# DanMcGann/loam

Hardware: AMD Instinct MI355X
Metric: scan-pair registrations/sec (64x1024 Ouster) (higher is better)
Workload: dtype f64; 1 GPU; batch of 1024 independent 64x1024 scan pairs per GPU (BASELINE configs[2]/[3]); step = extractFeatures x2 + registerFeatures per pair, inputs resident in HBM; pairs_per_gpu=1024, scan=64x1024, seed=20240311, input_scalar=f64, arithmetic=f64 (float input is widened on load)

## Files before the change

### loam_amd/csrc/loamx_api.hip

```cpp
#include <math.h>
#include <stdio.h>
#include <stdlib.h>
#include <string.h>

#include <mutex>
#include <utility>
#include <string>
#include <vector>

#include <dlfcn.h>
#include <rccl/rccl.h>

#include "loamx_internal.h"
#include "synth.h"

using namespace loamx;

namespace {

enum WsId {
  WS_XYZ = 0, WS_CURV, WS_MASK, WS_EDGE_STAGE, WS_PLANAR_STAGE, WS_EDGE_CNT, WS_PLANAR_CNT,
  WS_EDGE_IDX, WS_PLANAR_IDX, WS_N_EDGE, WS_N_PLANAR, WS_EDGE_XYZ, WS_PLANAR_XYZ,
  WS_GRID_DESC_E, WS_GRID_DESC_P, WS_CELLS_E, WS_CELLS_P, WS_SORTED_E, WS_SORTED_P, WS_REL_E, WS_REL_P,
  WS_SGRID_DESC_E, WS_SGRID_DESC_P, WS_SCELLS_E, WS_SCELLS_P, WS_SSORTED_E, WS_SSORTED_P, WS_SORT_SCRATCH, WS_SORT_SCRATCH_SRC, WS_ASSOC_E, WS_ASSOC_P, WS_NN_E, WS_NN_P, WS_RNN_E, WS_RNN_P, WS_NEAREST_E, WS_NEAREST_P, WS_REST_E, WS_REST_P, WS_EXACT_E, WS_EXACT_P, WS_NASSOC, WS_STATE, WS_PARTIALS, WS_MOM_PARTIALS, WS_MOMENTS, WS_FLAGGED_LIST, WS_FLAGGED_COUNT, WS_LINE_TOT, WS_EXTRACT_EVENTS, WS_BOX, WS_FINITE_FLAG,
  WS_COUNTERS, WS_ITERINFO, WS_STREAM_IN0, WS_STREAM_IN1, WS_STREAM_RES, WS_DUMP_E, WS_DUMP_P, WS_FIT_IN, WS_FIT_OUT, WS_SRC_E, WS_SRC_P, WS_TGT_E, WS_TGT_P, WS_FCOUNTS, WS_RESULTS, WS_INIT,
  WS_COUNT
};

struct Buf {
  void* p = nullptr;
  size_t cap = 0;
};

struct PendingEvent {
  int kernel;
  hipEvent_t e0, e1;
  double bytes;
  bool own_e0;
};

}

struct loamx_ctx {
  int device = 0;
  hipStream_t own_stream = nullptr, stream = nullptr;
  bool max_counts_clean = false;
  hipStream_t aux_stream = nullptr;
  hipEvent_t ev_fork = nullptr, ev_mid = nullptr, ev_join = nullptr;
  hipEvent_t ev_counts = nullptr;
  hipStream_t aux2_stream = nullptr;
  hipEvent_t ev_join2 = nullptr;
  std::string last_error;
  Buf ws[WS_COUNT];
  uint32_t* h_pinned = nullptr;
  bool timing = false;
  std::vector<PendingEvent> pending;
  std::vector<hipEvent_t> event_pool;
  hipEvent_t tail_event = nullptr;
  bool tail_fresh = false;
  loamx_kernel_stat stats[LOAMX_K_COUNT] = {};

  uint32_t extract_flags = 0;
  uint32_t reg_flags = 0;
  int map_cells_log2 = 0;
  int stream_chunk_pairs = 0;
  hipStream_t copy_stream = nullptr;
  hipEvent_t ev_up[2] = {nullptr, nullptr}, ev_free[2] = {nullptr, nullptr};

  unsigned long long sweep_slots_base[2] = {0, 0};
  unsigned long long features_base = 0;
  std::mutex mu;
};

struct loamx_target_index {
  GridDesc* desc[2] = {nullptr, nullptr};
  uint32_t* cells[2] = {nullptr, nullptr};
  GridPoint* sorted[2] = {nullptr, nullptr};
  float* rel[2] = {nullptr, nullptr};
  double* pts[2] = {nullptr, nullptr};
  size_t n[2] = {0, 0};
  size_t cap[2] = {0, 0};
  double radius[2] = {0, 0};
  uint32_t* counts = nullptr;
  void* scratch = nullptr;
  uint32_t cells_cap[2] = {0, 0};
  size_t cells_alloc[2] = {0, 0}, scratch_alloc = 0;
  GridPoint* sorted2[2] = {nullptr, nullptr};
  float* rel2[2] = {nullptr, nullptr};
  size_t n_at_build[2] = {0, 0};
  bool grid_valid[2] = {false, false};
  uint64_t full_builds = 0, merges = 0;
};

namespace loamx {
thread_local LaunchScope* g_launch_scope = nullptr;
int g_debug_sync = getenv("LOAMX_DEBUG_SYNC") ? 1 : 0;
}

namespace {

const char* kKernelNames[LOAMX_K_COUNT] = {"curvature_valid_kernel", "select_kernel", "compact_kernel",
                                           "grid_build_kernel",      "associate_kernel", "sweep_kernel",
                                           "lm_kernels",             "moment_kernel",    "knn_plane_kernel",
                                           "extract_fused_kernel"};

struct OptionName {
  const char* name;
  bool extract;
  uint32_t bit;
};
const OptionName kOptionNames[] = {
    {"FORCE_TIE_REPLAY", true, kFlagForceReplay}, {"FORCE_SCAN_GIVEUP", true, kFlagForceGiveUp}, {"CURV_V1", true, kFlagCurvV1},
    {"NO_FUSED_COMPACT", true, kFlagNoFusedCompact}, {"NO_MIS_SELECT", true, kFlagNoMisSelect}, {"FUSED_EXTRACT", true, kFlagFusedExtract},
    {"NO_ROW_SELECT", true, kFlagNoRowSelect}, {"FUSED_ROWS", true, kFlagFusedRows}, {"NO_SPLIT_CURV", true, kFlagNoSplitCurv}, {"STAGE_ALWAYS", true, kFlagStageAlways},
    {"NO_MOMENTS", false, kRegFlagNoMoments}, {"NO_PACKED_GRID", false, kRegFlagNoPackedGrid}, {"NO_BIG_GRID", false, kRegFlagNoBigGrid},
    {"NO_GRID_SIDE", false, kRegFlagNoGridSide}, {"DEBUG_POISON", false, kRegFlagPoison},
    {"QUEUE_TWO_STAGE", false, kRegFlagQueueTwoStage}, {"QUEUE_ONE_STAGE", false, kRegFlagQueueOneStage},
    {"NO_MIXED_ASSOC", false, kRegFlagNoMixedAssoc}, {"FORCE_RCCL", false, kRegFlagForceRccl},
    {"NO_COOP_LEFT", false, kRegFlagNoCoopLeft}, {"NO_REF_MOMENTS", false, kRegFlagNoRefMoments},
    {"NO_EXTRACT_BOXES", false, kRegFlagNoExtractBoxes}, {"CHECK_FINITE", false, kRegFlagCheckFinite},
    {"NO_SMALL_SETS", false, kRegFlagNoSmallSets}};

int fail(loamx_ctx* ctx, int code, const std::string& msg) {
  if (ctx) ctx->last_error = msg;
  return code;
}

#define HIP_TRY(ctx, expr)                                                                          \
  do {                                                                                              \
    hipError_t e_ = (expr);                                                                         \
    if (e_ != hipSuccess)                                                                           \
      return fail(ctx, LOAMX_ERR_HIP, std::string(#expr) + ": " + hipGetErrorString(e_));           \
  } while (0)

int ensure(loamx_ctx* ctx, int id, size_t bytes) {
  Buf& b = ctx->ws[id];
  if (bytes == 0) bytes = 8;
  if (b.cap >= bytes) return LOAMX_OK;
  if (b.p) {
    HIP_TRY(ctx, hipStreamSynchronize(ctx->stream));
    HIP_TRY(ctx, hipFree(b.p));
    b.p = nullptr, b.cap = 0;
  }
  HIP_TRY(ctx, hipMalloc(&b.p, bytes));
  b.cap = bytes;
  return LOAMX_OK;
}
#define ENSURE(ctx, id, bytes)                       \
  do {                                               \
    int rc_ = ensure(ctx, id, bytes);                \
    if (rc_ != LOAMX_OK) return rc_;                 \
  } while (0)

const char* const kNonFiniteMsg = "non-finite coordinate in the input (the reference's behaviour is undefined there)";
bool host_all_finite(const void* p, bool f32, size_t n_scalars) {
  if (!p) return true;
  if (f32) {
    const float* v = static_cast<const float*>(p);
    float acc = 0.0f;
    for (size_t i = 0; i < n_scalars; i++) acc += v[i] * 0.0f;
    return acc == 0.0f;
  }
  const double* v = static_cast<const double*>(p);
  double acc = 0.0;
  for (size_t i = 0; i < n_scalars; i++) acc += v[i] * 0.0;
  return acc == 0.0;
}
template <typename T>
T* wsp(loamx_ctx* ctx, int id) {
  return reinterpret_cast<T*>(ctx->ws[id].p);
}

hipEvent_t take_event(loamx_ctx* ctx) {
  if (!ctx->event_pool.empty()) {
    hipEvent_t e = ctx->event_pool.back();
    ctx->event_pool.pop_back();
    return e;
  }
  hipEvent_t e = nullptr;
  (void)hipEventCreate(&e);
  return e;
}

struct TimedScope {
  loamx_ctx* ctx;
  PendingEvent pe;
  bool on, attach;
  LaunchScope ls;
  TimedScope(loamx_ctx* c, int kernel, double bytes, bool attach_ = false) : ctx(c), on(c->timing), attach(attach_) {
    if (on) {
      pe.kernel = kernel, pe.bytes = bytes;
      if (attach) {
        pe.own_e0 = true;
        pe.e0 = take_event(ctx), pe.e1 = take_event(ctx);
        ls = LaunchScope{pe.e0, pe.e1, true};
        g_launch_scope = &ls;
        return;
      }
      pe.own_e0 = !(ctx->tail_fresh && ctx->tail_event);
      pe.e0 = pe.own_e0 ? take_event(ctx) : ctx->tail_event;
      pe.e1 = take_event(ctx);
      if (pe.own_e0) (void)hipEventRecord(pe.e0, ctx->stream);
    }
  }
// ... 278 lines not shown
    }
    if (it > 0 || ref_first) {
      TimedScope t(ctx, LOAMX_K_MOMENT, 0.0, true);
      launch_moments(B, s);
    }
    if (it > 0 || ref_first) {
      TimedScope t(ctx, LOAMX_K_LM, 0.0, true);
      launch_lm_pair_loop(B, C, s);
    } else {
      for (int k = 0; k < 5; k++) {
        {
          TimedScope t(ctx, LOAMX_K_SWEEP, 0.0, true);
          launch_sweep(B, s);
        }
        {
          TimedScope t(ctx, LOAMX_K_LM, 0.0, true);
          launch_lm_step(B, s);
        }
      }
    }
    CHECK_LAUNCH(ctx, "sweep/lm kernels");
    if (it == 0 && !ref_first) {
      TimedScope t(ctx, LOAMX_K_LM, 0.0, true);
      launch_outer_update(B, C, s);
    }
    CHECK_LAUNCH(ctx, "outer_update_kernel");
  return LOAMX_OK;
}

int register_dev(loamx_ctx* ctx, const RegInputs& in, const RegConfig& C_in, loamx_reg_result* d_results, bool want_iter_info,
                 AfterAssocHook hook, void* hook_user, const loamx_target_index* prebuilt = nullptr, const loamx_assoc_dump* dump = nullptr,
                 size_t dump_n_se = 0, size_t dump_n_sp = 0) {
  if (in.n_pairs == 0) return LOAMX_OK;
  RegConfig C = C_in;
  if (dump && C.max_iterations == 0) C.max_iterations = 1;
  untimed(ctx);
  if (in.n_pairs > 0x7FFFFFFFull / 128) return fail(ctx, LOAMX_ERR_UNSUPPORTED, "too many pairs in one call");
  const size_t np = in.n_pairs, es = in.edge_stride ? in.edge_stride : 1, ps = in.planar_stride ? in.planar_stride : 1;
  if (es > 0x3FFFFFFFull || ps > 0x3FFFFFFFull) return fail(ctx, LOAMX_ERR_UNSUPPORTED, "feature set too large");
  RegBatch B{};
  B.n_pairs = np, B.edge_stride = es, B.planar_stride = ps, B.in_pitch = in.in_pitch;
  B.src_edge = in.src_edge, B.n_src_edge = in.n_src_edge, B.src_planar = in.src_planar, B.n_src_planar = in.n_src_planar;
  B.tgt_edge = in.tgt_edge, B.n_tgt_edge = in.n_tgt_edge, B.tgt_planar = in.tgt_planar, B.n_tgt_planar = in.n_tgt_planar;
  B.init = in.init;
  if (!(C.flags & kRegFlagNoExtractBoxes)) B.box_min = in.boxes.min, B.box_max = in.boxes.max, B.box_bad = in.boxes.bad;
  ENSURE(ctx, WS_GRID_DESC_E, np * sizeof(GridDesc));
  ENSURE(ctx, WS_GRID_DESC_P, np * sizeof(GridDesc));
  ENSURE(ctx, WS_CELLS_E, (np * (size_t)(kGridCellsCap + 1) + 4) * sizeof(uint32_t));
  ENSURE(ctx, WS_CELLS_P, (np * (size_t)(kGridCellsCap + 1) + 4) * sizeof(uint32_t));
  ENSURE(ctx, WS_SORTED_E, np * (es + kGridPad) * sizeof(GridPoint));
  ENSURE(ctx, WS_SORTED_P, np * (ps + kGridPad) * sizeof(GridPoint));
  ENSURE(ctx, WS_REL_E, np * 3 * (es + kGridPad) * sizeof(float));
  ENSURE(ctx, WS_REL_P, np * 3 * (ps + kGridPad) * sizeof(float));
  ENSURE(ctx, WS_SGRID_DESC_E, np * sizeof(GridDesc));
  ENSURE(ctx, WS_SGRID_DESC_P, np * sizeof(GridDesc));
  ENSURE(ctx, WS_SCELLS_E, np * (size_t)(kGridCellsCap + 1) * sizeof(uint32_t));
  ENSURE(ctx, WS_SCELLS_P, np * (size_t)(kGridCellsCap + 1) * sizeof(uint32_t));
  ENSURE(ctx, WS_SSORTED_E, np * es * sizeof(GridPoint));
  ENSURE(ctx, WS_SSORTED_P, np * ps * sizeof(GridPoint));
  ENSURE(ctx, WS_SORT_SCRATCH, np * (es > ps ? es : ps) * sizeof(GridPoint));
  ENSURE(ctx, WS_SORT_SCRATCH_SRC, grid_small(es > ps ? es : ps, C.flags) ? sizeof(GridPoint) : np * (es > ps ? es : ps) * sizeof(GridPoint));
  ENSURE(ctx, WS_ASSOC_E, 9 * np * es * sizeof(double));
  ENSURE(ctx, WS_ASSOC_P, 7 * np * ps * sizeof(double));
  const size_t km_e = C.k_edge <= 5 ? 5 : (C.k_edge <= 8 ? 8 : kMaxK), km_p = C.k_plane <= 5 ? 5 : (C.k_plane <= 8 ? 8 : kMaxK);
  ENSURE(ctx, WS_NN_E, (1 + km_e) * np * es * sizeof(uint32_t));
  ENSURE(ctx, WS_NN_P, (1 + km_p) * np * ps * sizeof(uint32_t));
  ENSURE(ctx, WS_RNN_E, (1 + km_e) * np * es * sizeof(uint32_t));
  ENSURE(ctx, WS_RNN_P, (1 + km_p) * np * ps * sizeof(uint32_t));
  ENSURE(ctx, WS_NEAREST_E, np * es * sizeof(uint32_t));
  ENSURE(ctx, WS_NEAREST_P, np * ps * sizeof(uint32_t));
  ENSURE(ctx, WS_REST_E, np * es * sizeof(uint32_t));
  ENSURE(ctx, WS_REST_P, np * ps * sizeof(uint32_t));
  ENSURE(ctx, WS_EXACT_E, np * es * sizeof(uint32_t));
  ENSURE(ctx, WS_EXACT_P, np * ps * sizeof(uint32_t));
  ENSURE(ctx, WS_NASSOC, np * 8 * sizeof(uint32_t));
  ENSURE(ctx, WS_STATE, np * sizeof(PairState));
  B.blocks_per_pair = (uint32_t)((es + ps + kSweepChunk - 1) / kSweepChunk);
  ENSURE(ctx, WS_PARTIALS, np * B.blocks_per_pair * kAccSize * sizeof(double));
  B.mom_blocks_per_pair = (uint32_t)((ps + kSweepChunk - 1) / kSweepChunk);
  ENSURE(ctx, WS_MOM_PARTIALS, np * B.mom_blocks_per_pair * 4 * (size_t)(kMomSize + 2) * sizeof(double));
  ENSURE(ctx, WS_MOMENTS, np * (size_t)(kMomSize + 2) * sizeof(double));
  ENSURE(ctx, WS_FLAGGED_LIST, np * (size_t)B.mom_blocks_per_pair * kSweepChunk * sizeof(uint32_t));
  ENSURE(ctx, WS_FLAGGED_COUNT, np * (size_t)B.mom_blocks_per_pair * 4 * sizeof(uint32_t));
  {
    const bool fresh = ctx->ws[WS_COUNTERS].cap == 0;
    ENSURE(ctx, WS_COUNTERS, 128);
    untimed(ctx);
    if (fresh) HIP_TRY(ctx, hipMemsetAsync(ctx->ws[WS_COUNTERS].p, 0, 128, ctx->stream));
  }
  if (C.flags & kRegFlagPoison) {
    static const int kScratch[] = {WS_GRID_DESC_E, WS_GRID_DESC_P, WS_CELLS_E, WS_CELLS_P, WS_SORTED_E, WS_SORTED_P, WS_REL_E, WS_REL_P,
                                   WS_SGRID_DESC_E, WS_SGRID_DESC_P, WS_SCELLS_E, WS_SCELLS_P, WS_SSORTED_E, WS_SSORTED_P, WS_SORT_SCRATCH, WS_SORT_SCRATCH_SRC,
                                   WS_ASSOC_E, WS_ASSOC_P, WS_NN_E, WS_NN_P, WS_RNN_E, WS_RNN_P, WS_NEAREST_E, WS_NEAREST_P, WS_REST_E,
                                   WS_REST_P, WS_EXACT_E, WS_EXACT_P, WS_NASSOC, WS_STATE, WS_PARTIALS, WS_MOM_PARTIALS, WS_MOMENTS,
                                   WS_FLAGGED_LIST, WS_FLAGGED_COUNT};
    for (int id : kScratch)
      if (ctx->ws[id].p) HIP_TRY(ctx, hipMemsetAsync(ctx->ws[id].p, 0xFF, ctx->ws[id].cap, ctx->stream));
  }
  if (want_iter_info) ENSURE(ctx, WS_ITERINFO, np * (size_t)(C.max_iterations ? C.max_iterations : 1) * sizeof(loamx_iter_info));
  B.grid_edge = GridSet{wsp<GridDesc>(ctx, WS_GRID_DESC_E), wsp<uint32_t>(ctx, WS_CELLS_E), wsp<GridPoint>(ctx, WS_SORTED_E), es + kGridPad,
                        wsp<float>(ctx, WS_REL_E)};
  B.grid_plane = GridSet{wsp<GridDesc>(ctx, WS_GRID_DESC_P), wsp<uint32_t>(ctx, WS_CELLS_P), wsp<GridPoint>(ctx, WS_SORTED_P), ps + kGridPad,
                         wsp<float>(ctx, WS_REL_P)};
  B.src_grid_edge = GridSet{wsp<GridDesc>(ctx, WS_SGRID_DESC_E), wsp<uint32_t>(ctx, WS_SCELLS_E), wsp<GridPoint>(ctx, WS_SSORTED_E), es, nullptr};
  B.src_grid_plane = GridSet{wsp<GridDesc>(ctx, WS_SGRID_DESC_P), wsp<uint32_t>(ctx, WS_SCELLS_P), wsp<GridPoint>(ctx, WS_SSORTED_P), ps, nullptr};
  B.sort_scratch = wsp<GridPoint>(ctx, WS_SORT_SCRATCH);
  B.sort_scratch_src = wsp<GridPoint>(ctx, WS_SORT_SCRATCH_SRC);
  B.assoc = AssocBuffers{wsp<double>(ctx, WS_ASSOC_E), wsp<double>(ctx, WS_ASSOC_P), wsp<uint32_t>(ctx, WS_NN_E),
                         wsp<uint32_t>(ctx, WS_NN_P), wsp<uint32_t>(ctx, WS_RNN_E), wsp<uint32_t>(ctx, WS_RNN_P),
                         wsp<uint32_t>(ctx, WS_NEAREST_E),
                         wsp<uint32_t>(ctx, WS_NEAREST_P), wsp<uint32_t>(ctx, WS_REST_E), wsp<uint32_t>(ctx, WS_REST_P),
                         wsp<uint32_t>(ctx, WS_EXACT_E), wsp<uint32_t>(ctx, WS_EXACT_P),
                         wsp<uint32_t>(ctx, WS_NASSOC)};
  B.state = wsp<PairState>(ctx, WS_STATE);
  B.partials = wsp<double>(ctx, WS_PARTIALS);
  B.mom_partials = wsp<double>(ctx, WS_MOM_PARTIALS);
  B.moments = wsp<double>(ctx, WS_MOMENTS);
  B.flagged_list = wsp<uint32_t>(ctx, WS_FLAGGED_LIST);
  B.flagged_count = wsp<uint32_t>(ctx, WS_FLAGGED_COUNT);
  B.n_active = wsp<uint32_t>(ctx, WS_COUNTERS);
  B.sweep_slots = reinterpret_cast<unsigned long long*>(wsp<unsigned char>(ctx, WS_COUNTERS) + 8);
  B.assoc_slots = B.sweep_slots + 2;
  B.grid_bytes = B.sweep_slots + 5;
  B.iter_info = want_iter_info ? wsp<loamx_iter_info>(ctx, WS_ITERINFO) : nullptr;
  B.want_nearest = hook ? 1u : 0u;
  B.ref_moments = (C.flags & (kRegFlagNoMoments | kRegFlagNoRefMoments)) ? 0u : 1u;
  B.max_counts = wsp<uint32_t>(ctx, WS_COUNTERS) + 16;
  B.assoc_blocks_edge = B.assoc_blocks_plane = 0xFFFFFFFFu;
  B.knn_mode_edge = B.knn_mode_plane = 0u;
  B.small_edge_sets = (C.flags & kRegFlagNoSmallSets) ? 0u : (!prebuilt ? 1u : (prebuilt->n[0] <= kBruteMax ? 2u : 0u));
  hipStream_t s = ctx->stream;
  untimed(ctx);
  if (!ctx->max_counts_clean) {
    const uint32_t init[6] = {0u, 0u, 0u, 0u, 0xFFFFFFFFu, 0xFFFFFFFFu};
    memcpy(&ctx->h_pinned[8], init, sizeof(init));
    HIP_TRY(ctx, hipMemcpyAsync(B.max_counts, &ctx->h_pinned[8], sizeof(init), hipMemcpyHostToDevice, s));
  }
  ctx->max_counts_clean = false;
  launch_state_init(B, C, s);
  CHECK_LAUNCH(ctx, "state_init_kernel");
  if (!ctx->ev_counts) HIP_TRY(ctx, hipEventCreateWithFlags(&ctx->ev_counts, hipEventDisableTiming));
  HIP_TRY(ctx, hipMemcpyAsync(&ctx->h_pinned[16], B.max_counts, 6 * sizeof(uint32_t), hipMemcpyDeviceToHost, s));
  HIP_TRY(ctx, hipEventRecord(ctx->ev_counts, s));

  if (prebuilt) {
    B.grid_edge = GridSet{prebuilt->desc[0], prebuilt->cells[0], prebuilt->sorted[0], prebuilt->cap[0] + kGridPad, prebuilt->rel[0], prebuilt->cells_cap[0]};
    B.grid_plane = GridSet{prebuilt->desc[1], prebuilt->cells[1], prebuilt->sorted[1], prebuilt->cap[1] + kGridPad, prebuilt->rel[1], prebuilt->cells_cap[1]};
  }
  {
    TimedScope t(ctx, LOAMX_K_GRID, 0.0);
    const bool side = !(C.flags & kRegFlagNoGridSide) && ctx->aux_stream && !prebuilt && hipStreamWaitEvent(ctx->aux_stream, ctx->ev_counts, 0) == hipSuccess;
    if (!prebuilt) launch_grid_build_targets(B, C, s);
    launch_grid_build_sources(B, C, side ? ctx->aux_stream : s);
    if (side && hipEventRecord(ctx->ev_join, ctx->aux_stream) == hipSuccess) (void)hipStreamWaitEvent(s, ctx->ev_join, 0);
  }
  CHECK_LAUNCH(ctx, "grid_build_kernel");
  HIP_TRY(ctx, hipEventSynchronize(ctx->ev_counts));
  B.assoc_blocks_edge = (ctx->h_pinned[16] + 255u) / 256u;
  B.assoc_blocks_plane = (ctx->h_pinned[17] + 255u) / 256u;
  {
    uint32_t tmax[2] = {ctx->h_pinned[18], ctx->h_pinned[19]}, tmin[2] = {ctx->h_pinned[20], ctx->h_pinned[21]};
    if (prebuilt) tmax[0] = tmin[0] = (uint32_t)prebuilt->n[0], tmax[1] = tmin[1] = (uint32_t)prebuilt->n[1];
    uint32_t* mode[2] = {&B.knn_mode_edge, &B.knn_mode_plane};
    for (int k = 0; k < 2; k++) *mode[k] = tmin[k] > tmax[k] ? 0u : (tmin[k] > kBruteMax ? 1u : (tmax[k] <= kBruteMax ? 2u : 0u));
  }
  if (dump) {
    if (np != 1) return fail(ctx, LOAMX_ERR_BAD_PARAM, "association dump: one pair at a time");
    int rc_a = enqueue_association(ctx, B, C);
    if (rc_a != LOAMX_OK) return rc_a;
    untimed(ctx);
    const size_t n[2] = {dump_n_se, dump_n_sp}, kq[2] = {(size_t)C.k_edge, (size_t)C.k_plane}, pw[2] = {6, 4};
    AssocDumpSet D[2] = {};
    for (int kind = 0; kind < 2; kind++) {
      const size_t bytes = n[kind] * (24 + 8 * pw[kind] + 4 + 4 * kq[kind] + 1) + 64;
      ENSURE(ctx, kind ? WS_DUMP_P : WS_DUMP_E, bytes);
      unsigned char* base = wsp<unsigned char>(ctx, kind ? WS_DUMP_P : WS_DUMP_E);
      HIP_TRY(ctx, hipMemsetAsync(base, 0, bytes, s));
      D[kind].moved = reinterpret_cast<double*>(base);
      D[kind].prim = D[kind].moved + 3 * n[kind];
      D[kind].nn_count = reinterpret_cast<uint32_t*>(D[kind].prim + pw[kind] * n[kind]);
      D[kind].nn_idx = D[kind].nn_count + n[kind];
      D[kind].valid = reinterpret_cast<uint8_t*>(D[kind].nn_idx + kq[kind] * n[kind]);
      if (n[kind] == 0) D[kind].nn_count = nullptr;
    }
    launch_assoc_dump(B, C, D[0], D[1], s);
    CHECK_LAUNCH(ctx, "assoc_dump_kernel");
    struct Out { void* host; const void* dev; size_t bytes; };
    const Out outs[10] = {
        {dump->edge_nn_count, D[0].nn_count, 4 * n[0]}, {dump->edge_nn_idx, D[0].nn_idx, 4 * kq[0] * n[0]}, {dump->edge_valid, D[0].valid, n[0]},
        {dump->edge_moved, D[0].moved, 24 * n[0]}, {dump->edge_lines, D[0].prim, 48 * n[0]},
        {dump->plane_nn_count, D[1].nn_count, 4 * n[1]}, {dump->plane_nn_idx, D[1].nn_idx, 4 * kq[1] * n[1]}, {dump->plane_valid, D[1].valid, n[1]},
        {dump->plane_moved, D[1].moved, 24 * n[1]}, {dump->plane_planes, D[1].prim, 32 * n[1]}};
    for (const Out& o : outs)
      if (o.host && o.bytes && o.dev) HIP_TRY(ctx, hipMemcpyAsync(o.host, o.dev, o.bytes, hipMemcpyDeviceToHost, s));
    if (dump->queue_lengths) HIP_TRY(ctx, hipMemcpyAsync(dump->queue_lengths, B.assoc.n_assoc + 2, 4 * sizeof(uint32_t), hipMemcpyDeviceToHost, s));
    HIP_TRY(ctx, hipStreamSynchronize(s));
    return LOAMX_OK;
  }
  for (uint32_t it = 0; it < C.max_iterations; it++) {
    {
      const int rc_body = enqueue_icf_iteration(ctx, B, C, it, hook, hook_user);
      if (rc_body != LOAMX_OK) return rc_body;
    }
    if (it + 1 < C.max_iterations && it > (B.n_pairs >= 256 ? 1u : 0u)) {
      untimed(ctx);
      HIP_TRY(ctx, hipMemcpyAsync(ctx->h_pinned, B.n_active, sizeof(uint32_t), hipMemcpyDeviceToHost, s));
      launch_write_results(B, d_results, s);
      CHECK_LAUNCH(ctx, "write_results_kernel");
      HIP_TRY(ctx, hipStreamSynchronize(s));
      if (ctx->h_pinned[0] == 0) {
        ctx->max_counts_clean = true;
        return LOAMX_OK;
      }
    }
  }
  untimed(ctx);
  launch_write_results(B, d_results, s);
  CHECK_LAUNCH(ctx, "write_results_kernel");
  ctx->max_counts_clean = true;
  return LOAMX_OK;
}

int resolve_events(loamx_ctx* ctx) {
  if (ctx->pending.empty()) return LOAMX_OK;
  HIP_TRY(ctx, hipStreamSynchronize(ctx->stream));
  for (PendingEvent& pe : ctx->pending) {
    float ms = 0.f;
    if (hipEventElapsedTime(&ms, pe.e0, pe.e1) == hipSuccess) {
      ctx->stats[pe.kernel].launches++;
      ctx->stats[pe.kernel].total_ms += (double)ms;
      ctx->stats[pe.kernel].algorithmic_bytes += pe.bytes;
    }
    if (pe.own_e0) ctx->event_pool.push_back(pe.e0);
    ctx->event_pool.push_back(pe.e1);
  }
  ctx->pending.clear();
  ctx->tail_fresh = false;
  return LOAMX_OK;
}

}

extern "C" {

void loamx_default_fe_params(loamx_fe_params* p) { *p = loamx_fe_params{3, 6, 10, 50, 100.0, 1.0, 0.5, 1.0}; }
void loamx_default_reg_params(loamx_reg_params* p) {
  *p = loamx_reg_params{5, 1.0, 3, 10.0, 5, 2.0, 4, 0.1, 10, 1e-3, 1e-2, 100};
}

const char* loamx_status_string(int status) {
  switch (status) {
    case LOAMX_OK: return "ok";
    case LOAMX_ERR_SCAN_SIZE: return "LOAM: provided lidar scan size does not match provided lidar parameters";
    case LOAMX_ERR_BAD_PARAM: return "bad parameter";
    case LOAMX_ERR_HIP: return "HIP error";
    case LOAMX_ERR_CAPACITY: return "output capacity too small";
    case LOAMX_ERR_UNSUPPORTED: return "unsupported parameter combination";
    case LOAMX_ERR_NO_DEVICE: return "no usable HIP device";
    case LOAMX_ERR_COMM: return "RCCL error";
    default: return "unknown status";
  }
}

const char* loamx_last_error(const loamx_ctx* ctx) { return ctx ? ctx->last_error.c_str() : ""; }
const char* loamx_kernel_name(int id) { return (id >= 0 && id < LOAMX_K_COUNT) ? kKernelNames[id] : "?"; }

int loamx_ctx_create(int device, loamx_ctx** out) {
  if (!out) return LOAMX_ERR_BAD_PARAM;
  *out = nullptr;
  int n = 0;
  if (hipGetDeviceCount(&n) != hipSuccess || n <= 0 || device < 0 || device >= n) return LOAMX_ERR_NO_DEVICE;
  if (hipSetDevice(device) != hipSuccess) return LOAMX_ERR_NO_DEVICE;
  loamx_ctx* ctx = new loamx_ctx;
  ctx->device = device;
  if (hipStreamCreateWithFlags(&ctx->own_stream, hipStreamNonBlocking) != hipSuccess ||
      hipHostMalloc(reinterpret_cast<void**>(&ctx->h_pinned), 256, hipHostMallocDefault) != hipSuccess) {
    delete ctx;
    return LOAMX_ERR_HIP;
  }
  ctx->stream = ctx->own_stream;
  for (const OptionName& o : kOptionNames)
    if (getenv((std::string("LOAMX_") + o.name).c_str())) (o.extract ? ctx->extract_flags : ctx->reg_flags) |= o.bit;
  if (const char* mc = getenv("LOAMX_MAP_CELLS_LOG2")) ctx->map_cells_log2 = atoi(mc);
  if (const char* sc = getenv("LOAMX_STREAM_CHUNK_PAIRS")) ctx->stream_chunk_pairs = atoi(sc) > 0 ? atoi(sc) : 0;
  int prio_least = 0, prio_greatest = 0;
  (void)hipDeviceGetStreamPriorityRange(&prio_least, &prio_greatest);
  if (!getenv("LOAMX_NO_AUX_STREAM") &&
      hipStreamCreateWithPriority(&ctx->aux_stream, hipStreamNonBlocking, getenv("LOAMX_AUX_HIGH_PRIO") ? prio_greatest : prio_least) == hipSuccess) {
    if (hipEventCreateWithFlags(&ctx->ev_fork, hipEventDisableTiming) != hipSuccess ||
// ... 1212 lines not shown
```

### loam_amd/csrc/loamx_internal.h

```cpp
#pragma once
#include <hip/hip_runtime.h>
#include <hip/hip_ext.h>
#include <stdint.h>
#include <stdio.h>

#include "../../include/loamx.h"
#include "extract_math.h"
#include "reg_math.h"

namespace loamx {

struct LaunchScope {
  hipEvent_t start, stop;
  bool first;
};
extern thread_local LaunchScope* g_launch_scope;
extern int g_debug_sync;
template <typename F, typename... Args>
inline void launch_kernel_named(const char* name, F kernel, const dim3& grid, const dim3& block, size_t shmem, hipStream_t s, Args... args) {
  LaunchScope* sc = g_launch_scope;
  if (g_debug_sync) fprintf(stderr, "[loamx] launch %s grid %u x %u block %u\n", name, grid.x, grid.y, block.x), fflush(stderr);
  if (sc) {
    hipExtLaunchKernelGGL(kernel, grid, block, (uint32_t)shmem, s, sc->first ? sc->start : nullptr, sc->stop, 0, args...);
    sc->first = false;
// ... 8 lines not shown
#define launch_kernel(kernel, ...) launch_kernel_named(#kernel, kernel, __VA_ARGS__)

constexpr int kMaxNeighborPoints = 16;
constexpr int kMaxLineWidth = 4096;

struct ExtractStage {
  uint32_t* edge_stage;
  uint32_t* planar_stage;
  uint32_t* edge_cnt;
  uint32_t* planar_cnt;
};

struct ExtractFused {
  unsigned long long* line_tot;
  uint32_t fuse;
  const void* xyz;
  uint32_t f32;
  uint32_t* edge_idx;
  uint32_t* n_edge;
  double* edge_xyz;
  size_t edge_stride;
  uint32_t* planar_idx;
  uint32_t* n_planar;
  double* planar_xyz;
  size_t planar_stride;
  uint32_t* error;
  unsigned long long* events;
  unsigned long long* box_min;
  unsigned long long* box_max;
  uint32_t no_stage;
  const uint32_t* only_if;
};
__device__ __forceinline__ unsigned long long dbl_key(double v) {
  const unsigned long long u = (unsigned long long)__double_as_longlong(v);
  return (u >> 63) ? ~u : (u | 0x8000000000000000ull);
}
__device__ __forceinline__ double key_dbl(unsigned long long k) {
  return __longlong_as_double((long long)((k >> 63) ? (k & 0x7FFFFFFFFFFFFFFFull) : ~k));
}

void launch_curvature_valid(const void* d_xyz, bool f32, size_t n_scans, const ExtractParams& P, double* d_curv,
                            uint8_t* d_mask, hipStream_t s);
bool launch_select(const double* d_curv, const uint8_t* d_mask, size_t n_scans, const ExtractParams& P,
                   const ExtractStage& st, const ExtractFused* fz, hipStream_t s, bool* rows_ran = nullptr);
bool launch_select_takes_boxes(const ExtractParams& P);
bool launch_extract_fused(const void* d_xyz, bool f32, size_t n_scans, const ExtractParams& P, const ExtractStage& st,
                          const ExtractFused& fz, double* d_curv, uint8_t* d_mask, hipStream_t s);
bool launch_extract_rows_fused(const void* d_xyz, bool f32, size_t n_scans, const ExtractParams& P, const ExtractStage& st,
                               const ExtractFused& fz, double* d_curv, uint8_t* d_mask, hipStream_t s);
bool launch_extract_split_ok(const ExtractParams& P, size_t n_scans);
void launch_extract_init(unsigned long long* line_tot, size_t n_tot, unsigned long long* box_min, unsigned long long* box_max, size_t n_box,
                         hipStream_t s);
void launch_replay(const double* d_curv, const uint8_t* d_mask, size_t n_scans, const ExtractParams& P, const ExtractStage& st,
                   const ExtractFused& fz, hipStream_t s);
void launch_compact(const void* d_xyz, bool f32, size_t n_scans, const ExtractParams& P, const ExtractStage& st,
                    uint32_t* d_edge_idx, uint32_t* d_n_edge, double* d_edge_xyz, size_t edge_stride,
                    uint32_t* d_planar_idx, uint32_t* d_n_planar, double* d_planar_xyz, size_t planar_stride,
                    hipStream_t s, const uint32_t* only_if = nullptr, unsigned long long* fallback_counter = nullptr);

struct RegConfig {
  int k_edge, k_plane;
  int min_line_pts, min_plane_pts;
  double r_edge, r_plane;
  double pass_edge, pass_plane;
  double min_line_cond, max_avg_plane_dist;
  uint32_t max_iterations;
  double rot_thresh, pos_thresh;
  uint32_t min_associations;
  uint32_t flags;
};
constexpr uint32_t kRegFlagNoMoments = 1u;
constexpr uint32_t kRegFlagNoPackedGrid = 2u;
constexpr uint32_t kRegFlagNoBigGrid = 4u;
constexpr uint32_t kRegFlagNoGridSide = 8u;
constexpr uint32_t kRegFlagPoison = 16u;
constexpr uint32_t kRegFlagQueueTwoStage = 32u;
constexpr uint32_t kRegFlagQueueOneStage = 64u;
constexpr uint32_t kRegFlagForceRccl = 256u;
constexpr uint32_t kRegFlagNoCoopLeft = 512u;
constexpr uint32_t kRegFlagNoRefMoments = 1024u;
constexpr uint32_t kRegFlagNoSmallSets = 8192u;
constexpr uint32_t kRegFlagCheckFinite = 4096u;
constexpr uint32_t kRegFlagNoExtractBoxes = 2048u;
constexpr uint32_t kRegFlagNoMixedAssoc = 128u;

struct GridSet {
  GridDesc* desc;
  uint32_t* cell_start;
  GridPoint* sorted;
  size_t stride;
  float* rel;
  uint32_t cells_cap;
};

struct AssocBuffers {
  double* edge;
  double* plane;
  uint32_t* nn_edge;
  uint32_t* nn_plane;
  uint32_t* rnn_edge;
  uint32_t* rnn_plane;
  uint32_t* nearest_edge;
  uint32_t* nearest_plane;
  uint32_t* rest_edge;
  uint32_t* rest_plane;
  uint32_t* exact_edge;
  uint32_t* exact_plane;
  uint32_t* n_assoc;
};

struct PairState {
  double est[7];
  LmState lm;
  uint32_t active;
  uint32_t termination;
  uint32_t iterations;
  uint32_t first_sweep;
  uint32_t stream_planes;
  uint32_t use_moments;
  uint32_t mom_ref_on;
  double mom_ref[7];
};

constexpr int kSweepThreads = 256;
#ifndef LOAMX_SWEEP_ITEMS
#define LOAMX_SWEEP_ITEMS 16
#endif
constexpr int kSweepItems = LOAMX_SWEEP_ITEMS;
constexpr int kSweepChunk = kSweepThreads * kSweepItems;

struct RegBatch {
  size_t n_pairs;
  size_t edge_stride, planar_stride;
  uint32_t in_pitch;
  const double* src_edge;
  const uint32_t* n_src_edge;
  const double* src_planar;
  const uint32_t* n_src_planar;
  const double* tgt_edge;
  const uint32_t* n_tgt_edge;
  const double* tgt_planar;
  const uint32_t* n_tgt_planar;
  const double* init;
  GridSet grid_edge, grid_plane;
  GridSet src_grid_edge, src_grid_plane;
  GridPoint* sort_scratch;
  GridPoint* sort_scratch_src;
  AssocBuffers assoc;
  PairState* state;
  double* partials;
  double* mom_partials;
  double* moments;
  uint32_t mom_blocks_per_pair;
  uint32_t* flagged_list;
  uint32_t* flagged_count;
  uint32_t blocks_per_pair;
  uint32_t* n_active;
  unsigned long long* sweep_slots;
  unsigned long long* assoc_slots;
  unsigned long long* grid_bytes;
  loamx_iter_info* iter_info;
  uint32_t* max_counts;
  uint32_t knn_mode_edge, knn_mode_plane;
  uint32_t assoc_blocks_edge, assoc_blocks_plane;
  uint32_t want_nearest;
  uint32_t ref_moments;
  const unsigned long long* box_min;
  const unsigned long long* box_max;
  const uint32_t* box_bad;
  uint32_t small_edge_sets;
};

constexpr size_t kGridBigScratchBytes = 64 + ((size_t)kGridCellsCap + kGridCellsCap / 4096 + 8) * sizeof(uint32_t);
constexpr uint32_t kGridSmallCap = 20480;
constexpr uint32_t kBruteMax = 512;
constexpr uint32_t kGridMapCellsCap = 1u << 18;
inline bool grid_small(size_t stride, uint32_t reg_flags) { return stride <= kGridSmallCap && !(reg_flags & kRegFlagNoPackedGrid); }
void launch_grid_build_targets(const RegBatch& B, const RegConfig& C, hipStream_t s);
void launch_grid_build_sources(const RegBatch& B, const RegConfig& C, hipStream_t s);
void launch_grid_build_target(const RegBatch& B, const RegConfig& C, bool plane, hipStream_t s);
void launch_grid_build_source(const RegBatch& B, const RegConfig& C, bool plane, hipStream_t s);
void launch_state_init(const RegBatch& B, const RegConfig& C, hipStream_t s);
constexpr uint32_t kAssocEdges = 1u, kAssocPlanes = 2u;
void launch_associate(const RegBatch& B, const RegConfig& C, hipStream_t s, hipStream_t aux, hipStream_t aux2, hipEvent_t ev_fork,
                      hipEvent_t ev_mid, hipEvent_t ev_join, hipEvent_t ev_join2, LaunchScope* knn_scope = nullptr,
                      uint32_t what = kAssocEdges | kAssocPlanes);
#ifdef LOAMX_NN_SAME_STATS
void debug_nn_same(const RegBatch& B, uint32_t it, hipStream_t s);
#endif
void launch_lm_begin(const RegBatch& B, const RegConfig& C, hipStream_t s);
void launch_sweep(const RegBatch& B, hipStream_t s);
void launch_lm_pair_loop(const RegBatch& B, const RegConfig& C, hipStream_t s);
void launch_lm_step(const RegBatch& B, hipStream_t s);
void launch_moments(const RegBatch& B, hipStream_t s);
void launch_outer_update(const RegBatch& B, const RegConfig& C, hipStream_t s);
void launch_write_results(const RegBatch& B, loamx_reg_result* d_results, hipStream_t s);

size_t index_insert_ws_bytes(size_t cells, size_t n_add);
void launch_index_insert_count(const GridSet& gs, size_t cells, const double* d_add, uint32_t n_add, void* ws, hipStream_t s);
void launch_index_insert_merge(const GridSet& gs, size_t cells, uint32_t n_old, const double* d_add, uint32_t n_add, void* ws,
                               GridPoint* sorted2, float* rel2, hipStream_t s);

constexpr int kFitMaxK = 32;
struct AssocDumpSet {
  uint32_t* nn_count;
  uint32_t* nn_idx;
  uint8_t* valid;
  double* moved;
  double* prim;
};
void launch_fit_sets(bool plane, const double* d_pts, size_t n_sets, int k, double* d_prim, double* d_aux, hipStream_t s);
void launch_knn_queries(const GridSet& gs, const double* d_q, size_t n_q, int k, double max_dist, uint32_t* d_idx, uint32_t* d_count,
                        hipStream_t s);
void launch_assoc_dump(const RegBatch& B, const RegConfig& C, const AssocDumpSet& edge, const AssocDumpSet& plane, hipStream_t s);

void launch_check_finite(const void* d_pts, bool f32, const uint32_t* d_n, size_t n_sets, size_t stride, uint32_t pitch, uint32_t* d_flag,
                         hipStream_t s);
void launch_check_finite_scalars(const double* d_v, size_t n_scalars, uint32_t* d_flag, hipStream_t s);

void launch_synth_pairs(uint64_t seed, uint64_t first_pair, size_t n_pairs, uint32_t H, uint32_t W, double sigma,
                        double* d_xyz, hipStream_t s);

}
```

### loam_amd/csrc/reg_math.h

```cpp
#pragma once
#include <stdint.h>

#if defined(__HIPCC__)
#include <hip/hip_runtime.h>
#include <math.h>
#define LOAMX_HD __host__ __device__ __forceinline__
#else
#include <math.h>
#define LOAMX_HD inline
#endif

namespace loamx {

constexpr int kMaxK = 16;
constexpr double kDblMin = 2.2250738585072014e-308;
constexpr double kDblMax = 1.7976931348623157e308;
constexpr double kDblEps = 2.220446049250313e-16;

struct Vec3 {
  double x, y, z;
};
LOAMX_HD Vec3 v3(double x, double y, double z) { return Vec3{x, y, z}; }
LOAMX_HD Vec3 vadd(Vec3 a, Vec3 b) { return Vec3{a.x + b.x, a.y + b.y, a.z + b.z}; }
LOAMX_HD Vec3 vsub(Vec3 a, Vec3 b) { return Vec3{a.x - b.x, a.y - b.y, a.z - b.z}; }
// ... 832 lines not shown
        guard = d < guard ? d : guard;
      }
      if (c3[ax] + 1 < n3[ax] - 1) {
        const double d = ((o3[ax] + (double)(c3[ax] + 2) * g.h) - q3[ax]) * (1.0 - 1e-9) - m;
        guard = d < guard ? d : guard;
      }
    }
    if (guard < 0.0) guard = 0.0;
    const bool done = guard == kDblMax || knn_bound32(c, a, imask) < guard * guard || (max_dist > 0.0 && guard >= max_dist);
    if (!done) return -1;
  }
  uint32_t wbegin[KM], wts[KM];
#pragma unroll
  for (int i = 0; i < KM; i++) wbegin[i] = 0u, wts[i] = 0u;
  for (int rr = 0; rr < nrow; rr++) {
    const uint32_t w0 = row_scratch[(2 * rr) * row_stride] & 0x0FFFFFFFu, w1 = row_scratch[(2 * rr + 1) * row_stride];
    const uint32_t rts = w1 & 0x7FFFFFFFu;
    const bool visited = (w1 & 0x80000000u) != 0u;
#pragma unroll
    for (int i = 0; i < KM; i++) {
      const uint32_t tb = (c.key[i] & imask) >> 2;
      const bool take = visited && rts <= tb && rts >= wts[i];
      wbegin[i] = take ? w0 : wbegin[i];
      wts[i] = take ? rts : wts[i];
    }
  }
  int count = 0, kept = 0;
  bool undecided = false, open = true;
  double prev = -1.0, d5 = 0.0;
#pragma unroll
  for (int i = 0; i < KM; i++) {
    const uint32_t key = c.key[i];
    const bool real = i >= KM - k && key != 0xFFFFFFFFu;
    if (real) {
      if (key >= 0x7F800000u) undecided = true;
      const uint32_t tb = (key & imask) >> 2, ii = key & 3u;
      const uint32_t pp = wbegin[i] + (tb - wts[i]) * 4u + ii;
      pos[i] = pp;
      const GridPoint tp = sp[pp];
      const double dx = q.x - tp.x, dy = q.y - tp.y, dz = q.z - tp.z;
      const double d2 = dx * dx + dy * dy + dz * dz;
      if (!(d2 > prev)) undecided = true;
      if (!(d2 <= kDblMax)) undecided = true;
      prev = d2, d5 = d2;
      count++;
      if (open) {
        if (d2 <= pass_max) kept++;
        else open = false;
      }
    }
  }
  const uint32_t k6 = c.key[KM];
  if (count == k && k6 != 0xFFFFFFFFu) {
    const double t6 = (double)knn_bits_f32(k6 & ~imask);
    const double err = 2.0 * (3.4641016151377544 * a * sqrt(d5) + 3.0 * a * a + 2.384185791015625e-7 * d5);
    if (!(t6 > d5 + err)) undecided = true;
  }
  return undecided ? -1 : kept;
}


#if defined(LOAMX_KNN_STATS)
#define LOAMX_LEAN_REASON(r) (g_lean_reason = (r))
#else
#define LOAMX_LEAN_REASON(r) ((void)0)
#endif
constexpr int kLeanRowWords = 18;
#ifndef LOAMX_LEAN_TMAX
#define LOAMX_LEAN_TMAX 64
#endif
constexpr uint32_t kLeanMaxPoints = 65535u;

LOAMX_HD int knn_popcount64(uint64_t v) {
#if defined(__HIP_DEVICE_COMPILE__)
  return __popcll(v);
#else
  return __builtin_popcountll(v);
#endif
}

template <int KM, int W = 1>
LOAMX_HD int knn_lean_finish(const GridDesc& g, const GridPoint* __restrict__ sp, Vec3 q, int k, double max_dist, double pass_max,
                             double a, int32_t cx, int32_t cy, int32_t cz, const KnnKeys32<KM>& c, uint64_t started,
                             const uint32_t* row_scratch, int row_stride, int vis_off, uint32_t pos[KM]) {
  constexpr uint32_t imask = 0xFFu;
  constexpr int NR = (2 * W + 1) * (2 * W + 1);
  {
    double guard = kDblMax;
    const double m = 1e-9 * g.h;
    const int32_t c3[3] = {cx, cy, cz}, n3[3] = {g.nx, g.ny, g.nz};
    const double q3[3] = {q.x, q.y, q.z}, o3[3] = {g.ox, g.oy, g.oz};
#pragma unroll
    for (int ax = 0; ax < 3; ax++) {
      if (c3[ax] - W > 0) {
        const double d = (q3[ax] - (o3[ax] + (double)(c3[ax] - W) * g.h)) * (1.0 - 1e-9) - m;
        guard = d < guard ? d : guard;
      }
      if (c3[ax] + W < n3[ax] - 1) {
        const double d = ((o3[ax] + (double)(c3[ax] + W + 1) * g.h) - q3[ax]) * (1.0 - 1e-9) - m;
        guard = d < guard ? d : guard;
      }
    }
    if (guard < 0.0) guard = 0.0;
    const bool done = guard == kDblMax || knn_bound32(c, a, imask) < guard * guard || (max_dist > 0.0 && guard >= max_dist);
    if (!done) { LOAMX_LEAN_REASON(1); return -1; }
  }
  int count = 0, kept = 0;
  bool undecided = false, open = true;
  double prev = -1.0, d5 = 0.0;
  uint32_t vrow[KM];
#pragma unroll
  for (int i = 0; i < KM; i++) {
    const uint32_t tb = (c.key[i] & imask) >> 2;
    const int ord = knn_popcount64(started & ((2ull << tb) - 1ull)) - 1;
    vrow[i] = row_scratch[(vis_off + (ord < 0 ? 0 : (ord > NR - 1 ? NR - 1 : ord))) * row_stride];
  }
  GridPoint tp[KM];
#pragma unroll
  for (int i = 0; i < KM; i++) {
    const uint32_t key = c.key[i];
    const bool real = i >= KM - k && key != 0xFFFFFFFFu;
    const uint32_t tb = (key & imask) >> 2, ii = key & 3u;
    const uint32_t pp = real ? (vrow[i] & 0xFFFFu) + (tb - (vrow[i] >> 16)) * 4u + ii : 0u;
    pos[i] = pp;
    tp[i] = sp[pp < g.n_points ? pp : 0u];
  }
#pragma unroll
  for (int i = 0; i < KM; i++) {
    const uint32_t key = c.key[i];
    const bool real = i >= KM - k && key != 0xFFFFFFFFu;
    if (real) {
      if (key >= 0x7F800000u) undecided = true;
      const double dx = q.x - tp[i].x, dy = q.y - tp[i].y, dz = q.z - tp[i].z;
      const double d2 = dx * dx + dy * dy + dz * dz;
      if (!(d2 > prev)) undecided = true;
      if (!(d2 <= kDblMax)) undecided = true;
      prev = d2, d5 = d2;
      count++;
      if (open) {
        if (d2 <= pass_max) kept++;
        else open = false;
      }
    }
  }
  const uint32_t k6 = c.key[KM];
  if (count == k && k6 != 0xFFFFFFFFu) {
    const double t6 = (double)knn_bits_f32(k6 & ~imask);
#if defined(__HIP_DEVICE_COMPILE__)
    const double sd5 = (double)(__fsqrt_rn((float)d5) * 1.000001f) + 1e-18;
#else
    const double sd5 = (double)(sqrtf((float)d5) * 1.000001f) + 1e-18;
#endif
    const double err = 2.0 * (3.4641016151377544 * a * sd5 + 3.0 * a * a + 2.384185791015625e-7 * d5);
    if (!(t6 > d5 + err)) undecided = true;
  }
  if (undecided) LOAMX_LEAN_REASON(2);
  return undecided ? -3 : kept;
}

struct LeanBatch {
  KnnF4 x, y, z;
  uint32_t n;
};

template <int KM, int NR = 9>
LOAMX_HD bool knn_lean_half_trip(KnnKeys32<KM>& c, LeanBatch& cur, LeanBatch& nxt, uint32_t tu, uint32_t& p, uint32_t& e, int& ri,
                                 int& nv, uint64_t& started, uint32_t& rw, uint32_t& rthr, int nrow, uint32_t* row_scratch,
                                 int row_stride, float qx, float qy, float qz, const float* __restrict__ rel_x,
                                 const float* __restrict__ rel_y, const float* __restrict__ rel_z, uint32_t keep) {
  const bool step = p >= e && ri < nrow;
  const bool take = step && c.key[KM - 1] >= rthr;
  if (take) {
    row_scratch[nv * row_stride] = (rw & 0xFFFFu) | ((tu + 1u) << 16);
    nv++;
    started |= 1ull << ((tu + 1u) & 63u);
  }
  p = take ? (rw & 0xFFFFu) : p, e = take ? (rw >> 16) : e;
  ri += step ? 1 : 0;
  {
    const int rr = ri < NR - 1 ? ri : NR - 1;
    rw = row_scratch[rr * row_stride], rthr = row_scratch[(NR + rr) * row_stride];
  }
  {
    const bool work = p < e;
    nxt.n = work ? e - p : 0u;
    const uint32_t off = (work ? p : 0u) << 2;
    nxt.x = *reinterpret_cast<const KnnF4*>(reinterpret_cast<const char*>(rel_x) + off);
    nxt.y = *reinterpret_cast<const KnnF4*>(reinterpret_cast<const char*>(rel_y) + off);
    nxt.z = *reinterpret_cast<const KnnF4*>(reinterpret_cast<const char*>(rel_z) + off);
    p += work ? 4u : 0u;
  }
  knn_collect_batch_f32<KM>(c, qx, qy, qz, cur.x, cur.y, cur.z, cur.n, tu << 2, keep);
  return nxt.n != 0u || ri < nrow;
}

struct KnnSameQuery {
  LOAMX_HD Vec3 operator()(const Vec3& q) const { return q; }
};
template <int KM, typename Requery = KnnSameQuery>
LOAMX_HD int knn_lean_round1(const GridDesc& g, const uint32_t* __restrict__ cell_start, const GridPoint* __restrict__ sp,
                             const float* __restrict__ rel, uint32_t plane, Vec3 q, int k, double max_dist, double pass_max,
                             uint32_t pos[KM], uint32_t* row_scratch, int row_stride, Requery requery = Requery()) {
#pragma unroll
  for (int j = 0; j < KM; j++) pos[j] = 0;
  if (g.n_points == 0 || k <= 0) return 0;
  if (k > KM) k = KM;
  const int32_t cx = grid_cell_coord(q.x, g.ox, g.inv_h);
  const int32_t cy = grid_cell_coord(q.y, g.oy, g.inv_h);
  const int32_t cz = grid_cell_coord(q.z, g.oz, g.inv_h);
  const int32_t out = grid_outside_distance(g, cx, cy, cz);
  if (max_dist > 0.0 && out >= 1 && (double)(out - 1) * g.h >= max_dist) return 0;
  if (out > 1) { LOAMX_LEAN_REASON(3); return -1; }
  const double a = knn_f32_err_unit(g);
  const double r2 = knn_radius_bound(max_dist);
  const float qx = (float)(q.x - g.ox), qy = (float)(q.y - g.oy), qz = (float)(q.z - g.oz);
  const float kDown = 0.99999f, kUp = 1.00001f;
  const double sy2m = slab_dist(q.y, g.oy, g.h, cy - 1), sy2p = slab_dist(q.y, g.oy, g.h, cy + 1);
  const double sz2m = slab_dist(q.z, g.oz, g.h, cz - 1), sz2p = slab_dist(q.z, g.oz, g.h, cz + 1);
  const float fy2[3] = {(float)(sy2m * sy2m) * kDown, 0.0f, (float)(sy2p * sy2p) * kDown};
  const float fz2[3] = {(float)(sz2m * sz2m) * kDown, 0.0f, (float)(sz2p * sz2p) * kDown};
  const float fr2 = r2 < 1e37 ? (float)r2 * kUp : 3.0e38f;
  const float fa2 = (float)(3003.0 * a * a) * kUp;
  int nrow = 0;
  {
    const int32_t xa = cx - 1 < 0 ? 0 : cx - 1, xb = cx + 1 > g.nx - 1 ? g.nx - 1 : cx + 1;
    uint32_t rb[9], re[9];
#pragma unroll
    for (int o = 0; o < 9; o++) {
      constexpr int kOrder[9] = {4, 1, 3, 5, 7, 0, 2, 6, 8};
      const int j = kOrder[o];
      const int32_t iy = cy + (j % 3) - 1, iz = cz + (j / 3) - 1;
      const bool ok = xa <= xb && iy >= 0 && iy <= g.ny - 1 && iz >= 0 && iz <= g.nz - 1;
      const uint32_t row = ok ? (uint32_t)((iz * g.ny + iy) * g.nx) : 0u;
      const CellStart4 c4 = cell_start4_at(cell_start, ok ? row + (uint32_t)xa : 0u);
      const int span = xb + 1 - xa;
      rb[o] = ok ? c4.v[0] : 0u;
      re[o] = ok ? (span == 1 ? c4.v[1] : (span == 2 ? c4.v[2] : c4.v[3])) : 0u;
    }
#pragma unroll
    for (int o = 0; o < 9; o++) {
      constexpr int kOrder[9] = {4, 1, 3, 5, 7, 0, 2, 6, 8};
      const int j = kOrder[o];
      const float s2 = fy2[j % 3] + fz2[j / 3];
      const float x = (s2 * 0.99799f - fa2) * kDown;
      const uint32_t thr = x > 0.0f ? (knn_f32_bits(x) & ~0xFFu) : 0u;
      if (rb[o] < re[o] && s2 <= fr2) {
        row_scratch[nrow * row_stride] = rb[o] | (re[o] << 16);
        row_scratch[(9 + nrow) * row_stride] = thr;
        nrow++;
      }
    }
  }
  KnnKeys32<KM> c;
  knn_init(c, k);
#ifndef LOAMX_LEAN_TMAX
#define LOAMX_LEAN_TMAX 64
#endif
  constexpr uint32_t imask = 0xFFu, tmax = LOAMX_LEAN_TMAX;
  static_assert(imask == 0xFFu, "the row thresholds above clear the same bits");
  const float* __restrict__ rel_x = rel;
  const float* __restrict__ rel_y = rel + (size_t)plane;
  const float* __restrict__ rel_z = rel + 2 * (size_t)plane;
  uint32_t p = 0, e = 0;
  int ri = 0, nv = 0;
  uint64_t started = 0;
#if defined(__HIP_DEVICE_COMPILE__)
  uint32_t keep;
  asm volatile("v_mov_b32 %0, 0xffffff00" : "=v"(keep));
#else
  const uint32_t keep = ~imask;
#endif
  uint32_t t = 0;
#if !defined(LOAMX_LEAN_UNPIPELINED)
  LeanBatch b0 = {}, b1 = {};
  uint32_t rw = row_scratch[0], rthr = row_scratch[9 * row_stride];
  bool more = true;
  for (; t < tmax; t += 2) {
#if defined(__HIP_DEVICE_COMPILE__)
    const uint32_t tu = (uint32_t)__builtin_amdgcn_readfirstlane((int)t);
#else
    const uint32_t tu = t;
#endif
    knn_lean_half_trip<KM>(c, b0, b1, tu, p, e, ri, nv, started, rw, rthr, nrow, row_scratch, row_stride, qx, qy, qz, rel_x, rel_y,
                           rel_z, keep);
    more = knn_lean_half_trip<KM>(c, b1, b0, tu + 1u, p, e, ri, nv, started, rw, rthr, nrow, row_scratch, row_stride, qx, qy, qz,
                                  rel_x, rel_y, rel_z, keep);
    if (!more) break;
  }
  if (more) return -2;
#else
  for (; t < tmax; t++) {
#if defined(__HIP_DEVICE_COMPILE__)
    const uint32_t tu = (uint32_t)__builtin_amdgcn_readfirstlane((int)t);
#else
    const uint32_t tu = t;
#endif
    const bool have = ri < nrow, step = p >= e && have;
    const int rr = have ? ri : 0;
    const uint32_t w = row_scratch[rr * row_stride], thr = row_scratch[(9 + rr) * row_stride];
    const bool take = step && c.key[KM - 1] >= thr;
    ri += step ? 1 : 0;
    p = take ? (w & 0xFFFFu) : p, e = take ? (w >> 16) : e;
    if (take) {
      row_scratch[nv * row_stride] = (w & 0xFFFFu) | (tu << 16);
      nv++;
      started |= 1ull << tu;
    }
    if (p >= e && ri >= nrow) break;
    if (p < e) {
      knn_scan_batch_f32_soa<KM>(c, qx, qy, qz, rel_x, rel_y, rel_z, p, e - p, tu << 2, keep);
      p += 4u;
    }
  }
#endif
#if defined(LOAMX_KNN_STATS)
  g_lean_trips = t, g_lean_nrow = (uint32_t)nrow, g_lean_taken = (uint32_t)nv;
#endif
#if defined(LOAMX_LEAN_UNPIPELINED)
  if (p < e || ri < nrow) return -2;
#endif
  {
    const Vec3 q2 = requery(q);
    const int32_t cx2 = grid_cell_coord(q2.x, g.ox, g.inv_h), cy2 = grid_cell_coord(q2.y, g.oy, g.inv_h), cz2 = grid_cell_coord(q2.z, g.oz, g.inv_h);
    return knn_lean_finish<KM>(g, sp, q2, k, max_dist, pass_max, a, cx2, cy2, cz2, c, started, row_scratch, row_stride, 0, pos);
  }
}


template <int W>
struct LeanRowOrder {
  static constexpr int D = 2 * W + 1, NR = D * D;
  int v[NR];
  static constexpr int key(int j) { return (j % D - W) * (j % D - W) + (j / D - W) * (j / D - W); }
  constexpr LeanRowOrder() : v() {
    for (int i = 0; i < NR; i++) v[i] = i;
    for (int i = 1; i < NR; i++) {
      const int x = v[i];
      int j = i - 1;
      while (j >= 0 && key(v[j]) > key(x)) { v[j + 1] = v[j]; j--; }
      v[j + 1] = x;
    }
  }
};
constexpr int kLean2Rows = 25, kLean2RowWords = 2 * kLean2Rows, kLean4Rows = 81, kLean4RowWords = 2 * kLean4Rows;
template <int KM, int W>
LOAMX_HD int knn_lean_block(const GridDesc& g, const uint32_t* __restrict__ cell_start, const GridPoint* __restrict__ sp,
                            const float* __restrict__ rel, uint32_t plane, Vec3 q, int k, double max_dist, double pass_max,
                            uint32_t pos[KM], uint32_t* row_scratch, int row_stride) {
  constexpr int D = 2 * W + 1, NR = D * D;
#pragma unroll
  for (int j = 0; j < KM; j++) pos[j] = 0;
  if (g.n_points == 0 || k <= 0) return 0;
  if (k > KM) k = KM;
  const int32_t cx = grid_cell_coord(q.x, g.ox, g.inv_h);
  const int32_t cy = grid_cell_coord(q.y, g.oy, g.inv_h);
  const int32_t cz = grid_cell_coord(q.z, g.oz, g.inv_h);
  const int32_t out = grid_outside_distance(g, cx, cy, cz);
  if (max_dist > 0.0 && out >= 1 && (double)(out - 1) * g.h >= max_dist) return 0;
  if (out > W) return -1;
  const double a = knn_f32_err_unit(g);
  const double r2 = knn_radius_bound(max_dist);
  const float qx = (float)(q.x - g.ox), qy = (float)(q.y - g.oy), qz = (float)(q.z - g.oz);
  const float kDown = 0.99999f, kUp = 1.00001f;
  float fy2[D], fz2[D];
#pragma unroll
  for (int d = 0; d < D; d++) {
    const double sy = d == W ? 0.0 : slab_dist(q.y, g.oy, g.h, cy + d - W), sz = d == W ? 0.0 : slab_dist(q.z, g.oz, g.h, cz + d - W);
    fy2[d] = (float)(sy * sy) * kDown, fz2[d] = (float)(sz * sz) * kDown;
  }
  const float fr2 = r2 < 1e37 ? (float)r2 * kUp : 3.0e38f;
  const float fa2 = (float)(3003.0 * a * a) * kUp;
  int nrow = 0;
  {
    const int32_t xa = cx - W < 0 ? 0 : cx - W, xb = cx + W > g.nx - 1 ? g.nx - 1 : cx + W;
    constexpr LeanRowOrder<W> order{};
#pragma unroll
    for (int o0 = 0; o0 < NR; o0 += D) {
      uint32_t rb[D], re[D];
#pragma unroll
      for (int u = 0; u < D; u++) {
        const int j = order.v[o0 + u];
        const int32_t iy = cy + (j % D) - W, iz = cz + (j / D) - W;
        const bool ok = xa <= xb && iy >= 0 && iy <= g.ny - 1 && iz >= 0 && iz <= g.nz - 1;
        const uint32_t row = ok ? (uint32_t)((iz * g.ny + iy) * g.nx) : 0u;
        rb[u] = cell_start_at(cell_start, ok ? row + (uint32_t)xa : 0u);
        re[u] = cell_start_at(cell_start, ok ? row + (uint32_t)xb + 1u : 0u);
        if (!ok) rb[u] = re[u] = 0u;
      }
#pragma unroll
      for (int u = 0; u < D; u++) {
        const int j = order.v[o0 + u];
        const float s2 = fy2[j % D] + fz2[j / D];
        const float x = (s2 * 0.99799f - fa2) * kDown;
        const uint32_t thr = x > 0.0f ? (knn_f32_bits(x) & ~0xFFu) : 0u;
        if (rb[u] < re[u] && s2 <= fr2) {
          row_scratch[nrow * row_stride] = rb[u] | (re[u] << 16);
          row_scratch[(NR + nrow) * row_stride] = thr;
          nrow++;
        }
      }
    }
  }
  KnnKeys32<KM> c;
  knn_init(c, k);
  constexpr uint32_t tmax = 64;
  const float* __restrict__ rel_x = rel;
  const float* __restrict__ rel_y = rel + (size_t)plane;
  const float* __restrict__ rel_z = rel + 2 * (size_t)plane;
  uint32_t p = 0, e = 0;
  int ri = 0, nv = 0;
  uint64_t started = 0;
#if defined(__HIP_DEVICE_COMPILE__)
  uint32_t keep;
  asm volatile("v_mov_b32 %0, 0xffffff00" : "=v"(keep));
#else
  const uint32_t keep = ~0xFFu;
#endif
  LeanBatch b0 = {}, b1 = {};
  uint32_t rw = row_scratch[0], rthr = row_scratch[NR * row_stride];
  bool more = true;
  uint32_t t = 0;
  for (; t < tmax; t += 2) {
#if defined(__HIP_DEVICE_COMPILE__)
    const uint32_t tu = (uint32_t)__builtin_amdgcn_readfirstlane((int)t);
#else
    const uint32_t tu = t;
#endif
    knn_lean_half_trip<KM, NR>(c, b0, b1, tu, p, e, ri, nv, started, rw, rthr, nrow, row_scratch, row_stride, qx, qy, qz, rel_x, rel_y,
                               rel_z, keep);
    more = knn_lean_half_trip<KM, NR>(c, b1, b0, tu + 1u, p, e, ri, nv, started, rw, rthr, nrow, row_scratch, row_stride, qx, qy, qz,
                                      rel_x, rel_y, rel_z, keep);
    if (!more) break;
  }
  if (more) return -2;
  return knn_lean_finish<KM, W>(g, sp, q, k, max_dist, pass_max, a, cx, cy, cz, c, started, row_scratch, row_stride, 0, pos);
}
template <int KM>
LOAMX_HD int knn_lean_round2(const GridDesc& g, const uint32_t* __restrict__ cell_start, const GridPoint* __restrict__ sp,
                             const float* __restrict__ rel, uint32_t plane, Vec3 q, int k, double max_dist, double pass_max,
                             uint32_t pos[KM], uint32_t* row_scratch, int row_stride) {
  return knn_lean_block<KM, 2>(g, cell_start, sp, rel, plane, q, k, max_dist, pass_max, pos, row_scratch, row_stride);
}

template <int KM, bool WIDE = false, typename Requery = KnnSameQuery>
LOAMX_HD int knn_search_f32_round1(const GridDesc& g, const uint32_t* __restrict__ cell_start,
                                   const GridPoint* __restrict__ sp, const float* __restrict__ rel, uint32_t plane, Vec3 q,
                                   int k, double max_dist, double pass_max, uint32_t pos[KM], uint32_t* row_scratch,
                                   int row_stride, Requery requery = Requery()) {
#if !defined(LOAMX_NO_LEAN_KNN)
  if (!WIDE && g.n_points <= kLeanMaxPoints)
    return knn_lean_round1<KM>(g, cell_start, sp, rel, plane, q, k, max_dist, pass_max, pos, row_scratch, row_stride, requery);
#endif
#pragma unroll
  for (int j = 0; j < KM; j++) pos[j] = 0;
  if (g.n_points == 0 || k <= 0) return 0;
  if (k > KM) k = KM;
  const int32_t cx = grid_cell_coord(q.x, g.ox, g.inv_h);
  const int32_t cy = grid_cell_coord(q.y, g.oy, g.inv_h);
  const int32_t cz = grid_cell_coord(q.z, g.oz, g.inv_h);
  const int32_t out = grid_outside_distance(g, cx, cy, cz);
  if (max_dist > 0.0 && out >= 1 && (double)(out - 1) * g.h >= max_dist) return 0;
  if (out > 1) return -1;
  uint32_t pop = 0;
  const int nrow = knn_round1_list(g, cell_start, cx, cy, cz, row_scratch, row_stride, &pop);
  const uint32_t slots = pop + 4u * (uint32_t)nrow + 4u;
  const int kept = knn_f32_round1_body<KM, WIDE>(g, sp, rel, plane, q, k, max_dist, pass_max, pos, row_scratch, row_stride, cx,
                                                 cy, cz, nrow, slots);
  return kept;
}

template <int KM>
LOAMX_HD int knn_search_positions(const GridDesc& g, const uint32_t* __restrict__ cell_start,
                                  const GridPoint* __restrict__ sp, Vec3 q, int k, double max_dist, double pass_max,
                                  uint32_t pos[KM], uint32_t* row_scratch, int row_stride, uint32_t* fallbacks = nullptr) {
  int kept = knn_search_keyed<KM>(g, cell_start, sp, q, k, max_dist, pass_max, pos, row_scratch, row_stride);
  if (kept < 0) {
    if (fallbacks) (*fallbacks)++;
    if (k > KM) k = KM;
    KnnResult<KM> r;
    kept = knn_search(g, cell_start, sp, q, k, max_dist, r, row_scratch, row_stride);
    knn_shift_positions<KM>(r.pos, k, pos);
  }
  return kept;
}

LOAMX_HD void jacobi_rotate(double& app, double& aqq, double& apq, double& arp, double& arq, double& vp0, double& vp1,
                            double& vp2, double& vq0, double& vq1, double& vq2) {
  if (apq == 0.0) return;
  const double theta = (aqq - app) / (2.0 * apq);
  const double t = (theta >= 0.0 ? 1.0 : -1.0) / (fabs(theta) + sqrt(theta * theta + 1.0));
  const double c = 1.0 / sqrt(t * t + 1.0), s = t * c;
  const double app_n = app - t * apq, aqq_n = aqq + t * apq;
  const double arp_n = c * arp - s * arq, arq_n = s * arp + c * arq;
  app = app_n, aqq = aqq_n, apq = 0.0, arp = arp_n, arq = arq_n;
  double a, b;
  a = vp0, b = vq0, vp0 = c * a - s * b, vq0 = s * a + c * b;
  a = vp1, b = vq1, vp1 = c * a - s * b, vq1 = s * a + c * b;
  a = vp2, b = vq2, vp2 = c * a - s * b, vq2 = s * a + c * b;
}

template <int KM>
LOAMX_HD void fit_line(const Vec3 pts[KM], int K, Vec3& a, Vec3& b) {
  Vec3 sum = v3(0, 0, 0);
#pragma unroll
  for (int i = 0; i < KM; i++)
    if (i < K) sum = vadd(sum, pts[i]);
  const Vec3 center = v3(sum.x / (double)K, sum.y / (double)K, sum.z / (double)K);
  double a00 = 0, a11 = 0, a22 = 0, a01 = 0, a02 = 0, a12 = 0;
#pragma unroll
  for (int i = 0; i < KM; i++) {
    if (i < K) {
      const Vec3 d = vsub(pts[i], center);
      a00 += d.x * d.x, a11 += d.y * d.y, a22 += d.z * d.z;
      a01 += d.x * d.y, a02 += d.x * d.z, a12 += d.y * d.z;
    }
  }
  double v00 = 1, v01 = 0, v02 = 0, v10 = 0, v11 = 1, v12 = 0, v20 = 0, v21 = 0, v22 = 1;
  for (int sweep = 0; sweep < 32; sweep++) {
    if (a01 == 0.0 && a02 == 0.0 && a12 == 0.0) break;
    jacobi_rotate(a00, a11, a01, a02, a12, v00, v10, v20, v01, v11, v21);
    jacobi_rotate(a00, a22, a02, a01, a12, v00, v10, v20, v02, v12, v22);
    jacobi_rotate(a11, a22, a12, a01, a02, v01, v11, v21, v02, v12, v22);
  }
  int c0 = 0, c1 = 1, c2 = 2;
  double e0 = a00, e1 = a11, e2 = a22;
  {
    int k = 0;
    if (e1 < e0) k = 1;
    if (e2 < (k == 1 ? e1 : e0)) k = 2;
    if (k == 1) { double t = e0; e0 = e1; e1 = t; int ti = c0; c0 = c1; c1 = ti; }
    if (k == 2) { double t = e0; e0 = e2; e2 = t; int ti = c0; c0 = c2; c2 = ti; }
  }
  if (e2 < e1) { int ti = c1; c1 = c2; c2 = ti; }
  (void)c0, (void)c1, (void)e0;
// ... 586 lines not shown
}

LOAMX_HD double gradient_max_norm(const LmState& st) {
  double neg[6], xp[7];
  #pragma unroll
  for (int j = 0; j < 6; j++) neg[j] = -st.g[j];
  manifold_plus(st.x, neg, xp);
  double m = 0;
  #pragma unroll
  for (int i = 0; i < 7; i++) {
    const double a = fabs(st.x[i] - xp[i]);
    m = a > m ? a : m;
  }
  return m;
}

LOAMX_HD void lm_consume(LmState& st, const double acc[kAccSize], bool first) {
  const bool eval_ok = (acc[28] == 0.0);
  if (first) {
    if (!eval_ok) {
      st.active = 0;
      return;
    }
    #pragma unroll
    for (int j = 0; j < 21; j++) st.H[j] = acc[j];
    #pragma unroll
    for (int j = 0; j < 6; j++) st.g[j] = acc[21 + j];
    st.x_cost = acc[27];
    st.minimum_cost = st.x_cost;
    #pragma unroll
    for (int j = 0; j < 6; j++) st.scaling[j] = 1.0 / (1.0 + sqrt(sym_at(st.H, j, j)));
    st.active = lm_propose(st) ? 1 : 0;
    return;
  }
  const double cand_cost = eval_ok ? acc[27] : kDblMax;
  double step_norm = 0;
  #pragma unroll
  for (int i = 0; i < 7; i++) step_norm += (st.x[i] - st.xeval[i]) * (st.x[i] - st.xeval[i]);
  step_norm = sqrt(step_norm);
  if (step_norm <= 1e-8 * (st.x_norm + 1e-8)) {
    st.active = 0;
    return;
  }
  if (fabs(st.x_cost - cand_cost) <= 1e-6 * st.x_cost) {
    st.active = 0;
    return;
  }
  const double relative_decrease = (st.x_cost - cand_cost) / st.model_cost_change;
  if (relative_decrease > 1e-3) {
    #pragma unroll
    for (int i = 0; i < 7; i++) st.x[i] = st.xeval[i];
    double n2 = 0;
    #pragma unroll
    for (int i = 0; i < 7; i++) n2 += st.x[i] * st.x[i];
    st.x_norm = sqrt(n2);
    #pragma unroll
    for (int j = 0; j < 21; j++) st.H[j] = acc[j];
    #pragma unroll
    for (int j = 0; j < 6; j++) st.g[j] = acc[21 + j];
    st.x_cost = acc[27];
    double q = 2.0 * relative_decrease - 1.0;
    q = 1.0 - q * q * q;
    st.radius = st.radius / (q > 1.0 / 3.0 ? q : 1.0 / 3.0);
    st.radius = st.radius < 1e16 ? st.radius : 1e16;
    st.decrease_factor = 2.0;
    st.reuse_diagonal = 0;
    if (st.x_cost < st.minimum_cost) {
      st.minimum_cost = st.x_cost;
      #pragma unroll
      for (int i = 0; i < 7; i++) st.x_user[i] = st.x[i];
    }
    if (st.iteration < 4 && gradient_max_norm(st) <= 1e-10) {
      st.active = 0;
      return;
    }
  } else {
    st.radius = st.radius / st.decrease_factor;
    st.decrease_factor *= 2.0;
    st.reuse_diagonal = 1;
  }
  st.active = lm_propose(st) ? 1 : 0;
}

LOAMX_HD bool outer_update(double est[7], const double update[7], double rot_thresh, double pos_thresh) {
  double next[7];
  pose_compose(update, est, next);
  for (int i = 0; i < 7; i++) est[i] = next[i];
  const double angle_change = quat_angle_to_identity(update);
  const double position_change = sqrt(update[4] * update[4] + update[5] * update[5] + update[6] * update[6]);
  return angle_change < rot_thresh && position_change < pos_thresh;
}

}
```

### loam_amd/csrc/register_kernels.hip

```cpp
#include "loamx_internal.h"

namespace loamx {

namespace {

__device__ __forceinline__ double wave_min(double v) {
#pragma unroll
  for (int off = 32; off >= 1; off >>= 1) v = fmin(v, __shfl_xor(v, off));
  return v;
}
__device__ __forceinline__ double wave_max(double v) {
#pragma unroll
  for (int off = 32; off >= 1; off >>= 1) v = fmax(v, __shfl_xor(v, off));
  return v;
}

#ifndef LOAMX_BUILD_THREADS
#define LOAMX_BUILD_THREADS 1024
#endif
constexpr int kBuildThreads = LOAMX_BUILD_THREADS;

template <bool ORDERED, bool PACKED>
__global__ __launch_bounds__(kBuildThreads) void grid_build_kernel(const double* __restrict__ pts_base,
                                                                   const uint32_t* __restrict__ n_pts, size_t stride,
// ... 507 lines not shown
    const uint32_t c = c0 + u;
    if (c < ncell) {
      shift[c] = run;
      cursor[c] = cell_start[c + 1] + run;
    } else if (c == ncell) {
      shift[c] = run;
    }
    run += cnt[u];
  }
}

__global__ __launch_bounds__(256) void index_insert_move_kernel(const GridDesc* __restrict__ desc, uint32_t n_old, size_t stride,
                                                                const GridPoint* __restrict__ sorted, const float* __restrict__ rel,
                                                                const uint32_t* __restrict__ shift, GridPoint* __restrict__ sorted2,
                                                                float* __restrict__ rel2) {
  const uint32_t p = blockIdx.x * 256 + threadIdx.x;
  if (p >= n_old) return;
  const GridDesc g = *desc;
  const GridPoint e = sorted[p];
  const uint32_t np = p + shift[grid_cell_of_point(g, v3(e.x, e.y, e.z))];
  sorted2[np] = e;
  rel2[np] = rel[p], rel2[stride + np] = rel[stride + p], rel2[2 * stride + np] = rel[2 * stride + p];
}

__global__ __launch_bounds__(256) void index_insert_scatter_kernel(const double* __restrict__ add, uint32_t n_add, uint32_t first_index,
                                                                   const GridDesc* __restrict__ desc, size_t stride,
                                                                   const uint32_t* __restrict__ cell_of, uint32_t* __restrict__ cursor,
                                                                   GridPoint* __restrict__ sorted2, float* __restrict__ rel2) {
  const uint32_t i = blockIdx.x * 256 + threadIdx.x;
  if (i >= n_add) return;
  const GridDesc g = *desc;
  const double x = add[3 * (size_t)i], y = add[3 * (size_t)i + 1], z = add[3 * (size_t)i + 2];
  const uint32_t pos = atomicAdd(&cursor[cell_of[i]], 1u);
  sorted2[pos] = GridPoint{x, y, z, first_index + i, 0u};
  rel2[pos] = (float)(x - g.ox), rel2[stride + pos] = (float)(y - g.oy), rel2[2 * stride + pos] = (float)(z - g.oz);
}

__global__ __launch_bounds__(256) void index_insert_table_kernel(GridDesc* __restrict__ desc, uint32_t* __restrict__ cell_start,
                                                                 const uint32_t* __restrict__ shift, uint32_t n_new, size_t stride,
                                                                 float* __restrict__ rel2) {
  const uint32_t ncell = (uint32_t)(desc->nx * desc->ny * desc->nz);
  const uint32_t c = blockIdx.x * 256 + threadIdx.x;
  if (c <= ncell) cell_start[c] += shift[c];
  if (c < kGridPad) rel2[n_new + c] = kRelPad, rel2[stride + n_new + c] = kRelPad, rel2[2 * stride + n_new + c] = kRelPad;
  if (c == 0) desc->n_points = n_new;
}

constexpr int kRankThreads = 256;
__global__ __launch_bounds__(kRankThreads) void grid_rank_kernel(const uint32_t* __restrict__ n_pts, size_t stride,
                                                                 uint32_t in_pitch, GridSet gs,
                                                                 const GridPoint* __restrict__ scratch, const uint32_t* __restrict__ small_if) {
  const size_t pair = blockIdx.y;
  if (small_if && small_if[pair * in_pitch] <= kBruteMax) return;
  const uint32_t n_raw = n_pts[pair * in_pitch];
  const uint32_t n = n_raw < stride ? n_raw : (uint32_t)stride;
  const uint32_t p = blockIdx.x * kRankThreads + threadIdx.x;
  if (p >= n) return;
  const GridDesc g = gs.desc[pair];
  const uint32_t* __restrict__ cs = gs.cell_start + pair * (size_t)(kGridCellsCap + 1);
  const GridPoint* __restrict__ src = scratch + pair * gs.stride;
  GridPoint* __restrict__ sp = gs.sorted + pair * gs.stride;
  const GridPoint e = src[p];
  const uint32_t cell = grid_morton_of_point(g, v3(e.x, e.y, e.z));
  const uint32_t b = cs[cell], en = cs[cell + 1];
  uint32_t rank = 0;
#pragma unroll 4
  for (uint32_t j = b; j < en; j++) rank += src[j].orig < e.orig ? 1u : 0u;
  sp[b + rank] = e;
}

__global__ void state_init_kernel(RegBatch B, RegConfig C) {
  const size_t pair = (size_t)blockIdx.x * blockDim.x + threadIdx.x;
  if (pair >= B.n_pairs) return;
  PairState& S = B.state[pair];
  for (int i = 0; i < 7; i++) S.est[i] = B.init ? B.init[pair * 7 + i] : (i == 3 ? 1.0 : 0.0);
  S.active = C.max_iterations > 0 ? 1u : 0u;
  S.termination = LOAMX_MAX_ITER;
  S.iterations = 0;
  S.first_sweep = 0;
  S.stream_planes = 1;
  S.use_moments = 0;
  S.mom_ref_on = 0;
  S.lm.active = 0;
  for (int c = 0; c < 6; c++) B.assoc.n_assoc[8 * pair + c] = 0;
  if (B.max_counts) {
    const uint32_t ne = B.n_src_edge[pair * B.in_pitch], np = B.n_src_planar[pair * B.in_pitch];
    atomicMax(&B.max_counts[0], ne < B.edge_stride ? ne : (uint32_t)B.edge_stride);
    atomicMax(&B.max_counts[1], np < B.planar_stride ? np : (uint32_t)B.planar_stride);
    if (B.n_tgt_edge && B.n_tgt_planar) {
      uint32_t te = B.n_tgt_edge[pair * B.in_pitch], tp = B.n_tgt_planar[pair * B.in_pitch];
      te = te < B.edge_stride ? te : (uint32_t)B.edge_stride, tp = tp < B.planar_stride ? tp : (uint32_t)B.planar_stride;
      atomicMax(&B.max_counts[2], te), atomicMax(&B.max_counts[3], tp);
      atomicMin(&B.max_counts[4], te), atomicMin(&B.max_counts[5], tp);
    }
  }
}

constexpr int kAssocThreads = 256;
#ifndef LOAMX_ASSOC_WAVES
#define LOAMX_ASSOC_WAVES 4
#endif
#ifndef LOAMX_KNN_REQUERY
#define LOAMX_KNN_REQUERY 1
#endif
#ifndef LOAMX_ASSOC_WAVES5
#define LOAMX_ASSOC_WAVES5 (LOAMX_KNN_REQUERY ? 6 : 4)
#endif

__device__ __forceinline__ bool xcd_pair_map(uint32_t block, uint32_t blocks_per_pair, size_t n_pairs, size_t& pair,
                                             uint32_t& chunk) {
  if (n_pairs < 8) {
    pair = block / blocks_per_pair;
    chunk = block % blocks_per_pair;
  } else {
    const uint32_t xcd = block & 7u, slot = block >> 3;
    pair = (size_t)xcd + 8u * (size_t)(slot / blocks_per_pair);
    chunk = slot % blocks_per_pair;
  }
  return pair < n_pairs;
}

constexpr int kBruteTile = 256;
constexpr size_t kBruteLdsBytes = (kBruteTile + kGridPad) * sizeof(GridPoint) + ((3 * (kBruteTile + kGridPad) * sizeof(float) + 31) / 32) * 32;

template <class Coll>
__device__ __forceinline__ void brute_scan_tile(Coll& c, int k, Vec3 q, const GridPoint* s_tile, uint32_t tile, uint32_t tn) {
  for (uint32_t u = 0; u < tn; u += 4) {
    const GridPoint t0 = s_tile[u], t1 = s_tile[u + 1], t2 = s_tile[u + 2], t3 = s_tile[u + 3];
    double dx = q.x - t0.x, dy = q.y - t0.y, dz = q.z - t0.z;
    const double d0 = dx * dx + dy * dy + dz * dz;
    dx = q.x - t1.x, dy = q.y - t1.y, dz = q.z - t1.z;
    const double d1 = dx * dx + dy * dy + dz * dz;
    dx = q.x - t2.x, dy = q.y - t2.y, dz = q.z - t2.z;
    const double d2 = dx * dx + dy * dy + dz * dz;
    dx = q.x - t3.x, dy = q.y - t3.y, dz = q.z - t3.z;
    const double d3 = dx * dx + dy * dy + dz * dz;
    knn_offer4(c, k, d0, d1, d2, d3, tile + u, tn - u, t0.orig, t1.orig, t2.orig, t3.orig);
  }
}

template <bool PLANE, int KM>
__device__ __forceinline__ void knn_brute_body(const RegBatch& B, const RegConfig& C, uint32_t blocks_per_pair, uint32_t block,
                                               GridPoint* s_tile) {
  size_t pair;
  uint32_t chunk;
  if (!xcd_pair_map(block, blocks_per_pair, B.n_pairs, pair, chunk)) return;
  const PairState& S = B.state[pair];
  if (!S.active) return;
  const GridSet& gs = PLANE ? B.grid_plane : B.grid_edge;
  const uint32_t n_tgt = gs.desc[pair].n_points;
  if (n_tgt > kBruteMax) return;
  const size_t stride = PLANE ? B.planar_stride : B.edge_stride;
  const uint32_t n_src = PLANE ? B.n_src_planar[pair * B.in_pitch] : B.n_src_edge[pair * B.in_pitch];
  if ((PLANE ? B.knn_mode_plane : B.knn_mode_edge) == 2u && chunk == 0 && threadIdx.x == 0 && B.assoc_slots)
    atomicAdd(&B.assoc_slots[PLANE ? 1 : 0], (unsigned long long)(n_src < stride ? n_src : stride));
  if (chunk * kAssocThreads >= n_src || chunk * kAssocThreads >= stride) return;
  const uint32_t i = chunk * kAssocThreads + threadIdx.x;
  const bool has = i < n_src && i < stride;
  const GridSet& src_gs = PLANE ? B.src_grid_plane : B.src_grid_edge;
  const GridPoint* __restrict__ sp = gs.sorted + pair * gs.stride;
  Vec3 p = v3(0, 0, 0);
  if (has) {
    const GridPoint sq = src_gs.sorted[pair * src_gs.stride + i];
    p = pose_act(S.est, v3(sq.x, sq.y, sq.z));
  }
  int k = PLANE ? C.k_plane : C.k_edge;
  k = k < KM ? k : KM;
  const double max_dist = PLANE ? C.r_plane : C.r_edge;
  uint32_t pos[KM];
#pragma unroll
  for (int j = 0; j < KM; j++) pos[j] = 0;
  int kept = 0;
  if (k > 0 && n_tgt > 0) {
    const double pass_max = PLANE ? C.pass_plane : C.pass_edge;
    kept = has ? -1 : 0;
    const GridDesc g = gs.desc[pair];
    if (gs.rel != nullptr && g.h > 0.0) {
      float* s_f = reinterpret_cast<float*>(s_tile + kBruteTile + kGridPad);
      constexpr int kRow = kBruteTile + kGridPad;
      const float* __restrict__ rel = gs.rel + pair * 3 * gs.stride;
      const double a = knn_f32_err_unit(g);
      const bool inside = has && grid_outside_distance(g, grid_cell_coord(p.x, g.ox, g.inv_h), grid_cell_coord(p.y, g.oy, g.inv_h),
                                                       grid_cell_coord(p.z, g.oz, g.inv_h)) <= 1;
      const float qx = (float)(p.x - g.ox), qy = (float)(p.y - g.oy), qz = (float)(p.z - g.oz);
      constexpr uint32_t imask = 0x1FFu;
      static_assert(kBruteMax <= 512, "nine position bits");
      KnnKeys32<KM> c;
      knn_init(c, k);
      for (uint32_t tile = 0; tile < n_tgt; tile += kBruteTile) {
        const uint32_t tn = n_tgt - tile < (uint32_t)kBruteTile ? n_tgt - tile : (uint32_t)kBruteTile;
        __syncthreads();
        for (uint32_t t = threadIdx.x; t < tn + kGridPad; t += kAssocThreads) {
          s_f[t] = rel[tile + t], s_f[kRow + t] = rel[gs.stride + tile + t], s_f[2 * kRow + t] = rel[2 * gs.stride + tile + t];
        }
        __syncthreads();
        if (inside)
          for (uint32_t u = 0; u < tn; u += 4)
            knn_collect_batch_f32<KM>(c, qx, qy, qz, *reinterpret_cast<const KnnF4*>(s_f + u), *reinterpret_cast<const KnnF4*>(s_f + kRow + u),
                                      *reinterpret_cast<const KnnF4*>(s_f + 2 * kRow + u), tn - u, tile + u, ~imask);
      }
      if (inside) {
        int count = 0, kk = 0;
        bool undecided = false, open = true;
        double prev = -1.0, d5 = 0.0;
        GridPoint tp[KM];
#pragma unroll
        for (int j = 0; j < KM; j++) {
          const uint32_t pp = c.key[j] & imask;
          pos[j] = j >= KM - k && c.key[j] != 0xFFFFFFFFu ? pp : 0u;
          tp[j] = sp[pp < n_tgt ? pp : 0u];
        }
#pragma unroll
        for (int j = 0; j < KM; j++) {
          const uint32_t key = c.key[j];
          if (j >= KM - k && key != 0xFFFFFFFFu) {
            if (key >= 0x7F800000u) undecided = true;
            const double dx = p.x - tp[j].x, dy = p.y - tp[j].y, dz = p.z - tp[j].z;
            const double d2 = dx * dx + dy * dy + dz * dz;
            if (!(d2 > prev) || !(d2 <= kDblMax)) undecided = true;
            prev = d2, d5 = d2;
            count++;
            if (open) {
              if (d2 <= pass_max) kk++;
              else open = false;
            }
          }
        }
        const uint32_t k6 = c.key[KM];
        if (count == k && k6 != 0xFFFFFFFFu) {
          const double t6 = (double)knn_bits_f32(k6 & ~imask);
          const double err = 2.0 * (3.4641016151377544 * a * sqrt(d5) + 3.0 * a * a + 2.384185791015625e-7 * d5);
          if (!(t6 > d5 + err)) undecided = true;
        }
        if (!undecided) kept = kk;
      }
    }
    if (__syncthreads_or(kept < 0)) {
      KnnKeys<KM> c;
      knn_init(c, k, n_tgt);
      for (uint32_t tile = 0; tile < n_tgt; tile += kBruteTile) {
        const uint32_t tn = n_tgt - tile < (uint32_t)kBruteTile ? n_tgt - tile : (uint32_t)kBruteTile;
        __syncthreads();
        for (uint32_t t = threadIdx.x; t < tn + kGridPad; t += kAssocThreads) s_tile[t] = sp[tile + t];
        __syncthreads();
        if (kept < 0) brute_scan_tile(c, k, p, s_tile, tile, tn);
      }
      if (kept < 0) kept = knn_keys_finish(c, k, pass_max, pos);
    }
    if (__syncthreads_or(kept < 0)) {
      KnnResult<KM> r;
      knn_init(r);
      for (uint32_t tile = 0; tile < n_tgt; tile += kBruteTile) {
        const uint32_t tn = n_tgt - tile < (uint32_t)kBruteTile ? n_tgt - tile : (uint32_t)kBruteTile;
        __syncthreads();
        for (uint32_t t = threadIdx.x; t < tn + kGridPad; t += kAssocThreads) s_tile[t] = sp[tile + t];
        __syncthreads();
        if (kept < 0) brute_scan_tile(r, k, p, s_tile, tile, tn);
      }
      if (kept < 0) {
        kept = knn_finish(r, k, max_dist);
        knn_shift_positions<KM>(r.pos, k, pos);
      }
    }
  }
  if (!has) return;
  const size_t field = B.n_pairs * stride, slot = pair * stride + i;
  uint32_t* __restrict__ nn = PLANE ? B.assoc.nn_plane : B.assoc.nn_edge;
  nn[slot] = (uint32_t)kept;
#pragma unroll
  for (int j = 0; j < KM; j++) nn[(1 + j) * field + slot] = pos[j];
}
template <bool PLANE, int KM>
__global__ __launch_bounds__(kAssocThreads) void associate_knn_brute_kernel(RegBatch B, RegConfig C, uint32_t blocks_per_pair) {
  __shared__ GridPoint s_tile[kBruteLdsBytes / sizeof(GridPoint)];
  knn_brute_body<PLANE, KM>(B, C, blocks_per_pair, blockIdx.x, s_tile);
}

constexpr uint32_t kQueueIndex = 0x3FFFFFFFu, kQueueWide = 0x80000000u, kQueueTied = 0x40000000u;

template <bool PLANE, int KM>
__device__ __forceinline__ void knn_round1_body(const RegBatch& B, const RegConfig& C, uint32_t blocks_per_pair, uint32_t block,
                                                uint32_t* s_rows) {
  size_t pair;
  uint32_t chunk;
  if (!xcd_pair_map(block, blocks_per_pair, B.n_pairs, pair, chunk)) return;
  const uint32_t i = chunk * kAssocThreads + threadIdx.x;
  const PairState& S = B.state[pair];
  if (!S.active) return;
  const size_t stride = PLANE ? B.planar_stride : B.edge_stride;
  const uint32_t n_src = PLANE ? B.n_src_planar[pair * B.in_pitch] : B.n_src_edge[pair * B.in_pitch];
  const GridSet& gs = PLANE ? B.grid_plane : B.grid_edge;
  const GridSet& src_gs = PLANE ? B.src_grid_plane : B.src_grid_edge;
  if (chunk == 0 && threadIdx.x == 0 && B.assoc_slots)
    atomicAdd(&B.assoc_slots[PLANE ? 1 : 0], (unsigned long long)(n_src < stride ? n_src : stride));
  const GridDesc g = gs.desc[pair];
  if (g.n_points <= kBruteMax) return;
  if (i >= n_src || i >= stride) return;
  const GridPoint sq = src_gs.sorted[pair * src_gs.stride + i];
  const Vec3 p = pose_act(S.est, v3(sq.x, sq.y, sq.z));
  const uint32_t* __restrict__ cs = gs.cell_start + pair * (size_t)(kGridCellsCap + 1);
  const GridPoint* __restrict__ sp = gs.sorted + pair * gs.stride;
  uint32_t pos[KM];
  const float* __restrict__ rel = gs.rel + pair * 3 * gs.stride;
#if LOAMX_KNN_REQUERY
  const GridPoint* __restrict__ src_pts = src_gs.sorted + pair * src_gs.stride;
  auto requery = [&](const Vec3&) -> Vec3 {
    uint32_t ii = i;
    asm volatile("" : "+v"(ii));
    const GridPoint s2 = src_pts[ii];
    return pose_act(S.est, v3(s2.x, s2.y, s2.z));
  };
  const int kept = knn_search_f32_round1<KM, false, decltype(requery)>(g, cs, sp, rel, (uint32_t)gs.stride, p, PLANE ? C.k_plane : C.k_edge,
                                             PLANE ? C.r_plane : C.r_edge, PLANE ? C.pass_plane : C.pass_edge, pos,
                                             s_rows + threadIdx.x, kAssocThreads, requery);
#else
  const int kept = knn_search_f32_round1<KM>(g, cs, sp, rel, (uint32_t)gs.stride, p, PLANE ? C.k_plane : C.k_edge,
                                             PLANE ? C.r_plane : C.r_edge, PLANE ? C.pass_plane : C.pass_edge, pos,
                                             s_rows + threadIdx.x, kAssocThreads);
#endif
  const size_t field = B.n_pairs * stride, slot = pair * stride + i;
  uint32_t* __restrict__ nn = PLANE ? B.assoc.nn_plane : B.assoc.nn_edge;
  nn[slot] = kept < 0 ? 0xFFFFFFFFu : (uint32_t)kept;
  if (kept < 0) {
    const uint32_t at = atomicAdd(&B.assoc.n_assoc[8 * pair + (PLANE ? 3 : 2)], 1u);
    (PLANE ? B.assoc.rest_plane : B.assoc.rest_edge)[pair * stride + at] = i | (kept == -2 ? kQueueWide : kept == -3 ? kQueueTied : 0u);
  }
#pragma unroll
  for (int j = 0; j < KM; j++) nn[(1 + j) * field + slot] = pos[j];
}
template <bool PLANE, int KM>
__global__ __launch_bounds__(kAssocThreads, KM <= 5 ? LOAMX_ASSOC_WAVES5 : LOAMX_ASSOC_WAVES) void associate_knn_kernel(RegBatch B, RegConfig C,
                                                                                         uint32_t blocks_per_pair) {
  __shared__ uint32_t s_rows[kLeanRowWords * kAssocThreads];
  knn_round1_body<PLANE, KM>(B, C, blocks_per_pair, blockIdx.x, s_rows);
}
template <int KME, int KMP>
__global__ __launch_bounds__(kAssocThreads, (KME <= 5 && KMP <= 5) ? LOAMX_ASSOC_WAVES5 : LOAMX_ASSOC_WAVES) void associate_knn_mixed_kernel(RegBatch B, RegConfig C, uint32_t blocks_edge,
                                                                                               uint32_t blocks_plane, uint32_t edge_blocks) {
  constexpr size_t kRowBytes = sizeof(uint32_t) * kLeanRowWords * kAssocThreads, kTileBytes = kBruteLdsBytes;
  __shared__ __attribute__((aligned(16))) unsigned char s_raw[kRowBytes > kTileBytes ? kRowBytes : kTileBytes];
  if (blockIdx.x < edge_blocks) knn_brute_body<false, KME>(B, C, blocks_edge, blockIdx.x, reinterpret_cast<GridPoint*>(s_raw));
  else knn_round1_body<true, KMP>(B, C, blocks_plane, blockIdx.x - edge_blocks, reinterpret_cast<uint32_t*>(s_raw));
}

#ifndef LOAMX_REST_THREADS
#define LOAMX_REST_THREADS 64
#endif
constexpr int kRestThreads = LOAMX_REST_THREADS;
__host__ __device__ inline bool queue_leftovers_coop(const RegConfig& C, bool plane) {
  return !(C.flags & kRegFlagNoCoopLeft) && (plane ? C.r_plane : C.r_edge) > 0.0;
}
#ifndef LOAMX_COOP_WAVES
#define LOAMX_COOP_WAVES 4
#endif
#ifndef LOAMX_REST_WAVES
#define LOAMX_REST_WAVES(KM) ((KM) <= 8 ? 3 : 2)
#endif
template <bool PLANE, int KM, bool ONE_STAGE>
__global__ __launch_bounds__(kRestThreads, LOAMX_REST_WAVES(KM)) void associate_knn_rest_kernel(RegBatch B, RegConfig C,
                                                                                              uint32_t blocks_per_pair) {
  constexpr bool one_stage = ONE_STAGE;
  size_t pair;
  uint32_t chunk0;
  if (!xcd_pair_map(blockIdx.x, blocks_per_pair, B.n_pairs, pair, chunk0)) return;
  const PairState& S = B.state[pair];
  if (!S.active) return;
  const uint32_t queued = B.assoc.n_assoc[8 * pair + (PLANE ? 3 : 2)];
  if (queued == 0u) return;
  __shared__ uint32_t s_rows[(ONE_STAGE ? kLeanRowWords : kLean2RowWords) * kRestThreads];
  const size_t stride = PLANE ? B.planar_stride : B.edge_stride;
  const size_t field = B.n_pairs * stride;
  uint32_t* __restrict__ rnn = PLANE ? B.assoc.rnn_plane : B.assoc.rnn_edge;
  const uint32_t* __restrict__ rest = (PLANE ? B.assoc.rest_plane : B.assoc.rest_edge) + pair * stride;
  uint32_t* __restrict__ left = (PLANE ? B.assoc.exact_plane : B.assoc.exact_edge) + pair * stride;
  const GridSet& gs = PLANE ? B.grid_plane : B.grid_edge;
  const GridSet& src_gs = PLANE ? B.src_grid_plane : B.src_grid_edge;
  const GridDesc g = gs.desc[pair];
  const uint32_t* __restrict__ cs = gs.cell_start + pair * (size_t)(kGridCellsCap + 1);
  const GridPoint* __restrict__ sp = gs.sorted + pair * gs.stride;
  const bool spread = B.n_pairs < 8 && (size_t)queued * 4 <= (size_t)blocks_per_pair * kRestThreads;
  const uint32_t t0 = spread ? chunk0 + blocks_per_pair * threadIdx.x : chunk0 * kRestThreads + threadIdx.x;
  const uint32_t dt = spread ? 0xFFFFFFFFu - t0 : blocks_per_pair * kRestThreads;
  const bool lean_set = g.n_points <= kLeanMaxPoints;
  const int kq = PLANE ? C.k_plane : C.k_edge;
  const double max_dist = PLANE ? C.r_plane : C.r_edge, pass_max = PLANE ? C.pass_plane : C.pass_edge;
  for (uint32_t t = t0; t < queued; t += dt) {
    const uint32_t entry = rest[t], i = entry & kQueueIndex;
    const size_t slot = pair * stride + t;
    uint32_t pos[KM];
#pragma unroll
    for (int j = 0; j < KM; j++) pos[j] = 0;
    int kept = -1;
    const bool coop = !one_stage && queue_leftovers_coop(C, PLANE);
    if (one_stage || (!(entry & kQueueTied) && ((lean_set && !(entry & kQueueWide)) || ((entry & kQueueWide) && !coop)))) {
      const GridPoint sq = src_gs.sorted[pair * src_gs.stride + i];
      const Vec3 p = pose_act(S.est, v3(sq.x, sq.y, sq.z));
      if (entry & kQueueWide)
        kept = knn_search_f32_round1<KM, true>(g, cs, sp, gs.rel + pair * 3 * gs.stride, (uint32_t)gs.stride, p, kq, max_dist, pass_max, pos,
                                                s_rows + threadIdx.x, kRestThreads);
      else if (!one_stage)
        kept = knn_lean_round2<KM>(g, cs, sp, gs.rel + pair * 3 * gs.stride, (uint32_t)gs.stride, p, kq, max_dist, pass_max, pos,
                                   s_rows + threadIdx.x, kRestThreads);
      if (one_stage && kept < 0)
        kept = knn_search_keyed<KM>(g, cs, sp, p, kq, max_dist, pass_max, pos, s_rows + threadIdx.x, kRestThreads);
    }
    rnn[slot] = (uint32_t)kept;
    if (kept < 0) left[atomicAdd(&B.assoc.n_assoc[8 * pair + (PLANE ? 5 : 4)], 1u)] = t;
#pragma unroll
    for (int j = 0; j < KM; j++) rnn[(1 + j) * field + slot] = pos[j];
  }
}

template <bool PLANE, int KM>
__global__ __launch_bounds__(kRestThreads, 5) void associate_knn_left_kernel(RegBatch B, RegConfig C,
                                                                                              uint32_t blocks_per_pair) {
  size_t pair;
  uint32_t chunk0;
  if (!xcd_pair_map(blockIdx.x, blocks_per_pair, B.n_pairs, pair, chunk0)) return;
  const PairState& S = B.state[pair];
  if (!S.active) return;
  const uint32_t listed = B.assoc.n_assoc[8 * pair + (PLANE ? 5 : 4)];
  if (listed == 0u) return;
  __shared__ uint32_t s_rows[kLeanRowWords * kRestThreads];
  const size_t stride = PLANE ? B.planar_stride : B.edge_stride;
  const size_t field = B.n_pairs * stride;
  uint32_t* __restrict__ rnn = PLANE ? B.assoc.rnn_plane : B.assoc.rnn_edge;
  const uint32_t* __restrict__ rest = (PLANE ? B.assoc.rest_plane : B.assoc.rest_edge) + pair * stride;
  const uint32_t* __restrict__ left = (PLANE ? B.assoc.exact_plane : B.assoc.exact_edge) + pair * stride;
  const GridSet& gs = PLANE ? B.grid_plane : B.grid_edge;
  const GridSet& src_gs = PLANE ? B.src_grid_plane : B.src_grid_edge;
  const GridDesc g = gs.desc[pair];
  const uint32_t* __restrict__ cs = gs.cell_start + pair * (size_t)(kGridCellsCap + 1);
  const GridPoint* __restrict__ sp = gs.sorted + pair * gs.stride;
  const bool spread = B.n_pairs < 8 && (size_t)listed * 4 <= (size_t)blocks_per_pair * kRestThreads;
  const uint32_t t0 = spread ? chunk0 + blocks_per_pair * threadIdx.x : chunk0 * kRestThreads + threadIdx.x;
  const uint32_t dt = spread ? 0xFFFFFFFFu - t0 : blocks_per_pair * kRestThreads;
  for (uint32_t t = t0; t < listed; t += dt) {
    const uint32_t qpos = left[t], i = rest[qpos] & kQueueIndex;
    const size_t slot = pair * stride + qpos;
    const GridPoint sq = src_gs.sorted[pair * src_gs.stride + i];
    const Vec3 p = pose_act(S.est, v3(sq.x, sq.y, sq.z));
    uint32_t pos[KM];
    const int kept = knn_search_keyed<KM>(g, cs, sp, p, PLANE ? C.k_plane : C.k_edge, PLANE ? C.r_plane : C.r_edge,
                                          PLANE ? C.pass_plane : C.pass_edge, pos, s_rows + threadIdx.x, kRestThreads);
    rnn[slot] = (uint32_t)kept;
#pragma unroll
    for (int j = 0; j < KM; j++) rnn[(1 + j) * field + slot] = pos[j];
  }
}

constexpr int32_t kCoopMaxShell = 64;

__device__ __forceinline__ double wave_min_all(double v) {
#pragma unroll
  for (int off = 32; off >= 1; off >>= 1) {
    const double o = __shfl_xor(v, off);
    v = knn_key_min(v, o);
  }
  return v;
}

template <int KM>
__device__ __forceinline__ int knn_coop_search(const GridDesc& g, const uint32_t* __restrict__ cell_start, const GridPoint* __restrict__ sp,
                                               Vec3 q, int k, double max_dist, double pass_max, uint32_t pos[KM]) {
  const int lane = threadIdx.x & 63;
#pragma unroll
  for (int j = 0; j < KM; j++) pos[j] = 0;
  if (g.n_points == 0 || k <= 0) return 0;
  if (k > KM) k = KM;
  const int32_t cx = grid_cell_coord(q.x, g.ox, g.inv_h), cy = grid_cell_coord(q.y, g.oy, g.inv_h), cz = grid_cell_coord(q.z, g.oz, g.inv_h);
  const int32_t out = grid_outside_distance(g, cx, cy, cz);
  if (max_dist > 0.0 && out >= 1 && (double)(out - 1) * g.h >= max_dist) return 0;
  int32_t W = 0x7FFFFFFF;
  if (max_dist > 0.0) {
    const double wf = ceil(max_dist * g.inv_h) + 1.0 + (double)out;
    if (wf < 1.0e6) W = (int32_t)wf;
  }
  if (W > kCoopMaxShell) {
    const int32_t span = (g.nx > g.ny ? (g.nx > g.nz ? g.nx : g.nz) : (g.ny > g.nz ? g.ny : g.nz)) + out;
    if (span > kCoopMaxShell) return -2;
    W = span;
  }
  const double r2 = knn_radius_bound(max_dist);
  double bound = r2;
  KnnKeys<KM> c;
  knn_init(c, k, g.n_points);
  bool done = false;
  double kth = knn_key_empty();
  bool fresh = false;
  for (int32_t w = 1; w <= W && !done; w++) {
    const int ring_rows = w == 1 ? 9 : 8 * w;
    const int inner_rows = w == 1 ? 0 : (2 * w - 1) * (2 * w - 1);
    const int pieces = ring_rows + 2 * inner_rows;
    for (int u0 = 0; u0 < pieces; u0 += 64) {
      uint32_t rb = 0, re = 0;
      double s2 = kDblMax;
      {
        const int u = u0 + lane;
        int32_t dy = 0, dz = 0, xlo = cx - w, xhi = cx + w;
        bool cap = false;
        if (w == 1) {
// ... 41 lines not shown
        }
      }
      unsigned long long rows = __ballot(rb < re);
      while (rows) {
        const int b = __ffsll(rows) - 1;
        rows &= rows - 1;
        const uint32_t begin = (uint32_t)__builtin_amdgcn_readlane((int)rb, b), end = (uint32_t)__builtin_amdgcn_readlane((int)re, b);
        const double rs2 = __hiloint2double(__builtin_amdgcn_readlane(__double2hiint(s2), b), __builtin_amdgcn_readlane(__double2loint(s2), b));
        if (rs2 > bound) continue;
        fresh = true;
        for (uint32_t p0 = begin; p0 < end; p0 += 64) {
          const uint32_t p = p0 + (uint32_t)lane;
          const bool real = p < end;
          const GridPoint t = sp[real ? p : begin];
          const double dx = q.x - t.x, dy = q.y - t.y, dz = q.z - t.z;
          const double d2 = dx * dx + dy * dy + dz * dz;
          knn_key_insert(c, knn_key_pack(d2, p, c.mask, real));
        }
        if (end - begin >= 256u) {
          const double wb = wave_min_all(knn_bound(c, k));
          bound = wb < bound ? wb : bound;
        }
      }
    }
    {
      if (fresh) {
      fresh = false;
      KnnKeys<KM> cc = c;
      kth = knn_key_empty();
      for (int t = 0; t < k; t++) {
        double head = knn_key_empty();
#pragma unroll
        for (int j = KM; j >= 0; j--)
          if (j >= KM - k) head = cc.key[j] < head ? cc.key[j] : head;
        const double best = wave_min_all(head);
        kth = best;
        if (head == best && best < knn_key_empty()) {
#pragma unroll
          for (int j = 0; j < KM; j++)
            if (j >= KM - k) cc.key[j] = cc.key[j + 1];
          cc.key[KM] = knn_key_empty();
        }
      }
      }
      KnnKeys<KM> probe;
      probe.mask = c.mask;
#pragma unroll
      for (int j = 0; j <= KM; j++) probe.key[j] = kth;
      if (kth < knn_key_empty()) {
        const double ub = knn_bound(probe, k);
        bound = ub < bound ? ub : bound;
      }
      done = knn_done(g, q, k, max_dist, cx, cy, cz, probe, w);
    }
  }
  if (!done) return -1;
  KnnKeys<KM> m;
  knn_init(m, k, g.n_points);
#pragma unroll
  for (int t = 0; t <= KM; t++) {
    if (t >= KM - k) {
      double head = knn_key_empty();
#pragma unroll
      for (int j = KM; j >= 0; j--)
        if (j >= KM - k) head = c.key[j] < head ? c.key[j] : head;
      const double best = wave_min_all(head);
      m.key[t] = best;
      if (head == best && best < knn_key_empty()) {
#pragma unroll
        for (int j = 0; j < KM; j++)
          if (j >= KM - k) c.key[j] = c.key[j + 1];
        c.key[KM] = knn_key_empty();
      }
    }
  }
  return knn_keys_finish(m, k, pass_max, pos);
}

static_assert(kRestThreads == 64, "associate_knn_coop_kernel is written for one wavefront per workgroup");
template <bool PLANE, int KM>
__global__ __launch_bounds__(kRestThreads, LOAMX_COOP_WAVES) void associate_knn_coop_kernel(RegBatch B, RegConfig C, uint32_t blocks_per_pair) {
  size_t pair;
  uint32_t chunk0;
  if (!xcd_pair_map(blockIdx.x, blocks_per_pair, B.n_pairs, pair, chunk0)) return;
  const PairState& S = B.state[pair];
  if (!S.active) return;
  const uint32_t listed = B.assoc.n_assoc[8 * pair + (PLANE ? 5 : 4)];
  if (listed == 0u) return;
  __shared__ uint32_t s_rows[kLeanRowWords];
  const size_t stride = PLANE ? B.planar_stride : B.edge_stride;
  const size_t field = B.n_pairs * stride;
  uint32_t* __restrict__ rnn = PLANE ? B.assoc.rnn_plane : B.assoc.rnn_edge;
  const uint32_t* __restrict__ rest = (PLANE ? B.assoc.rest_plane : B.assoc.rest_edge) + pair * stride;
  const uint32_t* __restrict__ left = (PLANE ? B.assoc.exact_plane : B.assoc.exact_edge) + pair * stride;
  const GridSet& gs = PLANE ? B.grid_plane : B.grid_edge;
  const GridSet& src_gs = PLANE ? B.src_grid_plane : B.src_grid_edge;
  const GridDesc g = gs.desc[pair];
  const uint32_t* __restrict__ cs = gs.cell_start + pair * (size_t)(kGridCellsCap + 1);
  const GridPoint* __restrict__ sp = gs.sorted + pair * gs.stride;
  const int kq = PLANE ? C.k_plane : C.k_edge;
  const double max_dist = PLANE ? C.r_plane : C.r_edge, pass_max = PLANE ? C.pass_plane : C.pass_edge;
  for (uint32_t t = chunk0; t < listed; t += blocks_per_pair) {
    const uint32_t qpos = left[t], i = rest[qpos] & kQueueIndex;
    const size_t slot = pair * stride + qpos;
    const GridPoint sq = src_gs.sorted[pair * src_gs.stride + i];
    const Vec3 p = pose_act(S.est, v3(sq.x, sq.y, sq.z));
    uint32_t pos[KM];
    int kept = knn_coop_search<KM>(g, cs, sp, p, kq, max_dist, pass_max, pos);
    if (kept == -2) {
      if ((threadIdx.x & 63) == 0) kept = knn_search_keyed<KM>(g, cs, sp, p, kq, max_dist, pass_max, pos, s_rows, 1);
      kept = __builtin_amdgcn_readfirstlane(kept);
#pragma unroll
      for (int j = 0; j < KM; j++) pos[j] = (uint32_t)__builtin_amdgcn_readfirstlane((int)pos[j]);
    }
    if ((threadIdx.x & 63) == 0) {
      rnn[slot] = (uint32_t)kept;
#pragma unroll
      for (int j = 0; j < KM; j++) rnn[(1 + j) * field + slot] = pos[j];
    }
  }
}

template <bool PLANE, int KM>
__device__ __forceinline__ void knn_exact_one(const RegBatch& B, const RegConfig& C, const PairState& S, size_t pair, uint32_t i,
                                              size_t slot, uint32_t* rnn, uint32_t* s_rows, int rows_stride) {
  const size_t stride = PLANE ? B.planar_stride : B.edge_stride;
  const size_t field = B.n_pairs * stride;
  const GridSet& gs = PLANE ? B.grid_plane : B.grid_edge;
  const GridSet& src_gs = PLANE ? B.src_grid_plane : B.src_grid_edge;
  const GridDesc g = gs.desc[pair];
  const uint32_t* __restrict__ cs = gs.cell_start + pair * (size_t)(kGridCellsCap + 1);
  const GridPoint* __restrict__ sp = gs.sorted + pair * gs.stride;
  int k = PLANE ? C.k_plane : C.k_edge;
  k = k < KM ? k : KM;
  const GridPoint sq = src_gs.sorted[pair * src_gs.stride + i];
  const Vec3 p = pose_act(S.est, v3(sq.x, sq.y, sq.z));
  KnnResult<KM> r;
  const int kept = knn_search(g, cs, sp, p, k, PLANE ? C.r_plane : C.r_edge, r, s_rows, rows_stride);
  uint32_t pos[KM];
  knn_shift_positions<KM>(r.pos, k, pos);
  rnn[slot] = (uint32_t)kept;
#pragma unroll
  for (int j = 0; j < KM; j++) rnn[(size_t)(1 + j) * field + slot] = pos[j];
}

template <bool PLANE, int KM, bool QUEUED = false>
__device__ __forceinline__ bool fit_one(const RegBatch& B, const RegConfig& C, const PairState& S, size_t pair, uint32_t i,
                                        const uint32_t* __restrict__ nnsrc, size_t nidx) {
  const size_t stride = PLANE ? B.planar_stride : B.edge_stride;
  const GridSet& gs = PLANE ? B.grid_plane : B.grid_edge;
  const GridSet& src_gs = PLANE ? B.src_grid_plane : B.src_grid_edge;
  const GridPoint sq = src_gs.sorted[pair * src_gs.stride + i];
  const Vec3 p = pose_act(S.est, v3(sq.x, sq.y, sq.z));
  const GridPoint* __restrict__ sp = gs.sorted + pair * gs.stride;
  const size_t field = B.n_pairs * stride, slot = pair * stride + i;
  const int kept = (int)nnsrc[nidx];
  const int kq = PLANE ? C.k_plane : C.k_edge;
  const int shift = KM - (kq < KM ? kq : KM);
  double prim[6] = {0, 0, 0, 0, 0, 0};
  uint32_t nearest = 0xFFFFFFFFu;
  bool valid = false;
  uint32_t at[KM];
#pragma unroll
  for (int j = 0; j < KM; j++) at[j] = shift + j < KM ? nnsrc[(size_t)(1 + shift + j) * field + nidx] : 0u;
  if (!QUEUED && kept == -1) return false;
  GridPoint tp[KM];
#pragma unroll
  for (int j = 0; j < KM; j++) tp[j] = sp[at[j] < (uint32_t)gs.stride ? at[j] : 0u];
  if (kept >= (PLANE ? C.min_plane_pts : C.min_line_pts)) {
    Vec3 nb[KM];
#pragma unroll
    for (int j = 0; j < KM; j++) nb[j] = j < kept ? v3(tp[j].x, tp[j].y, tp[j].z) : v3(0, 0, 0);
    if (kept > 0) nearest = tp[0].orig;
    if (PLANE) {
      Vec3 nrm;
      double d;
      const double avg = fit_plane<KM>(nb, kept, nrm, d);
      valid = !(avg > C.max_avg_plane_dist);
      prim[0] = nrm.x, prim[1] = nrm.y, prim[2] = nrm.z, prim[3] = d;
    } else {
      Vec3 a, b;
      fit_line<KM>(nb, kept, a, b);
      valid = !(kDblMax < C.min_line_cond);
      prim[0] = a.x, prim[1] = a.y, prim[2] = a.z, prim[3] = b.x, prim[4] = b.y, prim[5] = b.z;
    }
  }
  double* __restrict__ rec = PLANE ? B.assoc.plane : B.assoc.edge;
  rec[slot] = valid ? p.x : __longlong_as_double(0x7FF8000000000000ll);
  rec[field + slot] = p.y;
  rec[2 * field + slot] = p.z;
#pragma unroll
  for (int f = 0; f < (PLANE ? 4 : 6); f++) rec[(3 + f) * field + slot] = prim[f];
  if (B.want_nearest) (PLANE ? B.assoc.nearest_plane : B.assoc.nearest_edge)[pair * stride + sq.orig] = valid ? nearest : 0xFFFFFFFFu;
  return valid;
}

#ifndef LOAMX_FIT_WAVES
#define LOAMX_FIT_WAVES 4
#endif
template <bool PLANE, int KM>
__device__ __forceinline__ void fit_body(const RegBatch& B, const RegConfig& C, uint32_t blocks_per_pair, uint32_t block) {
  size_t pair;
  uint32_t chunk;
  if (!xcd_pair_map(block, blocks_per_pair, B.n_pairs, pair, chunk)) return;
  const uint32_t i = chunk * kAssocThreads + threadIdx.x;
  const PairState& S = B.state[pair];
  if (!S.active) return;
  const size_t stride = PLANE ? B.planar_stride : B.edge_stride;
  const uint32_t n_src = PLANE ? B.n_src_planar[pair * B.in_pitch] : B.n_src_edge[pair * B.in_pitch];
  const uint32_t* __restrict__ nn = PLANE ? B.assoc.nn_plane : B.assoc.nn_edge;
  bool valid = false;
  if (i < n_src && i < stride) valid = fit_one<PLANE, KM>(B, C, S, pair, i, nn, pair * stride + i);
  const unsigned long long m = __ballot(valid);
  if ((threadIdx.x & 63) == 0 && m) atomicAdd(&B.assoc.n_assoc[8 * pair + (PLANE ? 1 : 0)], (uint32_t)__popcll(m));
}
template <bool PLANE, int KM>
__global__ __launch_bounds__(kAssocThreads, LOAMX_FIT_WAVES) void associate_fit_kernel(RegBatch B, RegConfig C,
                                                                                        uint32_t blocks_per_pair) {
  fit_body<PLANE, KM>(B, C, blocks_per_pair, blockIdx.x);
}
template <int KME, int KMP>
__global__ __launch_bounds__(kAssocThreads, LOAMX_FIT_WAVES) void associate_fit_mixed_kernel(RegBatch B, RegConfig C, uint32_t blocks_edge,
                                                                                              uint32_t blocks_plane, uint32_t edge_blocks) {
  if (blockIdx.x < edge_blocks) fit_body<false, KME>(B, C, blocks_edge, blockIdx.x);
  else fit_body<true, KMP>(B, C, blocks_plane, blockIdx.x - edge_blocks);
}

template <bool PLANE, int KM>
__global__ __launch_bounds__(kRestThreads, 3) void associate_fit_queued_kernel(RegBatch B, RegConfig C, uint32_t blocks_per_pair) {
  size_t pair;
  uint32_t chunk0;
  if (!xcd_pair_map(blockIdx.x, blocks_per_pair, B.n_pairs, pair, chunk0)) return;
  const PairState& S = B.state[pair];
  if (!S.active) return;
  const uint32_t queued = B.assoc.n_assoc[8 * pair + (PLANE ? 3 : 2)];
  if (queued == 0u) return;
  __shared__ uint32_t s_rows[18 * kRestThreads];
  const size_t stride = PLANE ? B.planar_stride : B.edge_stride;
  uint32_t* rnn = PLANE ? B.assoc.rnn_plane : B.assoc.rnn_edge;
  const uint32_t* __restrict__ rest = (PLANE ? B.assoc.rest_plane : B.assoc.rest_edge) + pair * stride;
  uint32_t count = 0;
  for (uint32_t t = chunk0 * kRestThreads + threadIdx.x; t < queued; t += blocks_per_pair * kRestThreads) {
    const uint32_t i = rest[t] & kQueueIndex;
    if ((int)rnn[pair * stride + t] < 0)
      knn_exact_one<PLANE, KM>(B, C, S, pair, i, pair * stride + t, rnn, s_rows + threadIdx.x, kRestThreads);
    count += fit_one<PLANE, KM, true>(B, C, S, pair, i, rnn, pair * stride + t) ? 1u : 0u;
  }
#pragma unroll
  for (int off = 32; off >= 1; off >>= 1) count += __shfl_xor(count, off);
  if ((threadIdx.x & 63) == 0 && count) atomicAdd(&B.assoc.n_assoc[8 * pair + (PLANE ? 1 : 0)], count);
}

__global__ __launch_bounds__(64) void lm_begin_kernel(RegBatch B, RegConfig C) {
  const size_t pair = (size_t)blockIdx.x * blockDim.x + threadIdx.x;
  if (pair >= B.n_pairs) return;
  if (pair == 0) *B.n_active = 0u;
  PairState& S = B.state[pair];
  if (!S.active) return;
  const uint32_t iteration = S.iterations;
  const uint32_t ne = B.assoc.n_assoc[8 * pair], np = B.assoc.n_assoc[8 * pair + 1];
  for (int c = 0; c < 6; c++) B.assoc.n_assoc[8 * pair + c] = 0;
  if ((uint64_t)ne + np < C.min_associations) {
    S.termination = LOAMX_INSUFFICIENT_ASSOCIATIONS;
    S.active = 0;
    S.lm.active = 0;
    return;
  }
  lm_init(S.lm);
  S.first_sweep = 1;
  S.mom_ref_on = 0;
  if (B.iter_info) {
    loamx_iter_info& I = B.iter_info[pair * C.max_iterations + iteration];
    for (int i = 0; i < 7; i++) I.target_T_source_init[i] = S.est[i];
    I.n_edge_associations = ne;
    I.n_plane_associations = np;
  }
}

#ifndef LOAMX_SWEEP_WAVES
#define LOAMX_SWEEP_WAVES 3
#endif
__global__ __launch_bounds__(kSweepThreads, LOAMX_SWEEP_WAVES) void sweep_kernel(RegBatch B) {
  __shared__ double s_part[kSweepThreads / 64][kAccSize];
  const size_t pair = blockIdx.x / B.blocks_per_pair;
  const uint32_t blk = blockIdx.x % B.blocks_per_pair;
  const PairState& S = B.state[pair];
  if (!S.active || !S.lm.active) return;
  double x[7];
#pragma unroll
  for (int i = 0; i < 7; i++) x[i] = S.lm.xeval[i];
  const uint32_t n_se_raw = B.n_src_edge[pair * B.in_pitch], n_sp_raw = B.n_src_planar[pair * B.in_pitch];
  const uint32_t n_se = n_se_raw < B.edge_stride ? n_se_raw : (uint32_t)B.edge_stride;
  const uint32_t n_sp = n_sp_raw < B.planar_stride ? n_sp_raw : (uint32_t)B.planar_stride;
  const size_t efield = B.n_pairs * B.edge_stride, pfield = B.n_pairs * B.planar_stride;
  const double* __restrict__ E = B.assoc.edge + pair * B.edge_stride;
  const double* __restrict__ Pl = B.assoc.plane + pair * B.planar_stride;
  double acc[kAccSize];
#pragma unroll
  for (int j = 0; j < kAccSize; j++) acc[j] = 0.0;
  if (S.stream_planes == 0u) return;
  const uint32_t total = n_se + n_sp;
  const uint32_t base = blk * kSweepChunk;
  if (base >= total) return;
  if (blk == 0 && threadIdx.x == 0 && B.sweep_slots) {
    atomicAdd(&B.sweep_slots[0], (unsigned long long)n_se);
    atomicAdd(&B.sweep_slots[1], (unsigned long long)n_sp);
  }
  {
  struct Rec {
    double f[9];
    int kind;
  };
  auto load_rec = [&](uint32_t v) {
    Rec R;
    R.kind = 0;
#pragma unroll
    for (int f = 0; f < 9; f++) R.f[f] = 0.0;
    if (v < total) {
      if (v < n_se) {
        R.kind = 1;
#pragma unroll
        for (int f = 0; f < 9; f++) R.f[f] = E[f * efield + v];
      } else {
        const uint32_t q = v - n_se;
        R.kind = 2;
#pragma unroll
        for (int f = 0; f < 7; f++) R.f[f] = Pl[f * pfield + q];
      }
    }
    return R;
  };
  Rec cur = load_rec(base + threadIdx.x);
#pragma unroll 1
  for (int it = 0; it < kSweepItems; it++) {
    const Rec nxt = (it + 1 < kSweepItems) ? load_rec(base + (it + 1) * kSweepThreads + threadIdx.x) : Rec{{0, 0, 0, 0, 0, 0, 0, 0, 0}, 0};
    if (cur.kind != 0 && cur.f[0] == cur.f[0]) {
      double prim[6];
#pragma unroll
      for (int f = 0; f < 6; f++) prim[f] = cur.f[3 + f];
// ... 151 lines not shown
  return v;
}

__device__ __forceinline__ double stream_eval_wave(const RegBatch& B, size_t pair, const double x[7], uint32_t n_se, uint32_t n_sp) {
  const int lane = threadIdx.x;
  const size_t efield = B.n_pairs * B.edge_stride, pfield = B.n_pairs * B.planar_stride;
  const double* __restrict__ E = B.assoc.edge + pair * B.edge_stride;
  const double* __restrict__ Pl = B.assoc.plane + pair * B.planar_stride;
  double acc[kAccSize];
#pragma unroll
  for (int j = 0; j < kAccSize; j++) acc[j] = 0.0;
  for (uint32_t v = lane; v < n_se; v += 64) {
    const double f0 = E[v];
    if (f0 == f0) {
      double prim[6];
#pragma unroll
      for (int f = 0; f < 6; f++) prim[f] = E[(3 + f) * efield + v];
      residual_accumulate(false, v3(f0, E[efield + v], E[2 * efield + v]), prim, x, acc);
    }
  }
  for (uint32_t q = lane; q < n_sp; q += 64) {
    const double f0 = Pl[q];
    if (f0 == f0) {
      const double prim[6] = {Pl[3 * pfield + q], Pl[4 * pfield + q], Pl[5 * pfield + q], Pl[6 * pfield + q], 0.0, 0.0};
      residual_accumulate(true, v3(f0, Pl[pfield + q], Pl[2 * pfield + q]), prim, x, acc);
    }
  }
  double mine = 0.0;
#pragma unroll
  for (int j = 0; j < kAccSize; j++) {
    double v = acc[j];
#pragma unroll
    for (int off = 32; off >= 1; off >>= 1) v += __shfl_xor(v, off);
    if (lane == j) mine = v;
  }
  return mine;
}

__device__ __forceinline__ void lm_step_pair(const RegBatch& B, size_t pair, PairState& S, const double* acc) {
  const double* __restrict__ mom = B.moments + pair * (size_t)(kMomSize + 2);
  LmState lm = S.lm;
  const bool first = S.first_sweep != 0;
  lm_consume(lm, acc, first);
  S.lm = lm;
  S.first_sweep = 0;
  if (first && B.ref_moments && !S.use_moments && lm.active) {
    S.use_moments = 1u, S.mom_ref_on = 1u;
    for (int i = 0; i < 7; i++) S.mom_ref[i] = lm.xeval[i];
    S.stream_planes = 1u;
    return;
  }
  const bool valid = S.mom_ref_on ? plane_moments_valid_rel(mom[kMomSize], mom[kMomSize + 1], lm.xeval, S.mom_ref)
                                  : plane_moments_valid_at(mom[kMomSize], mom[kMomSize + 1], lm.xeval);
  S.stream_planes = (!S.use_moments || (lm.active && !valid)) ? 1u : 0u;
}

__global__ __launch_bounds__(64) void lm_step_kernel(RegBatch B) {
  const size_t pair = (size_t)blockIdx.x * blockDim.x + threadIdx.x;
  if (pair >= B.n_pairs) return;
  PairState& S = B.state[pair];
  if (!S.active || !S.lm.active) return;
  const uint32_t n_se_raw = B.n_src_edge[pair * B.in_pitch], n_sp_raw = B.n_src_planar[pair * B.in_pitch];
  const uint32_t n_se = n_se_raw < B.edge_stride ? n_se_raw : (uint32_t)B.edge_stride;
  const uint32_t n_sp = n_sp_raw < B.planar_stride ? n_sp_raw : (uint32_t)B.planar_stride;
  const uint32_t used = S.stream_planes ? (n_se + n_sp + kSweepChunk - 1) / kSweepChunk : 1u;
  double acc[kAccSize];
  for (int j = 0; j < kAccSize; j++) acc[j] = 0.0;
  for (uint32_t b = 0; b < used && b < B.blocks_per_pair; b++) {
    const double* __restrict__ p = B.partials + (pair * B.blocks_per_pair + b) * kAccSize;
    for (int j = 0; j < kAccSize; j++) acc[j] += p[j];
  }
  lm_step_pair(B, pair, S, acc);
}

__device__ __forceinline__ void outer_update_pair(const RegBatch& B, const RegConfig& C, size_t pair, PairState& S) {
  const uint32_t iteration = S.iterations;
  double upd[7];
  for (int i = 0; i < 7; i++) upd[i] = S.lm.x_user[i];
  if (B.iter_info) {
    loamx_iter_info& I = B.iter_info[pair * C.max_iterations + iteration];
    for (int i = 0; i < 7; i++) I.estimate_update[i] = upd[i];
  }
  S.iterations = iteration + 1;
  double est[7];
  for (int i = 0; i < 7; i++) est[i] = S.est[i];
  const bool converged = outer_update(est, upd, C.rot_thresh, C.pos_thresh);
  S.use_moments = (C.flags & kRegFlagNoMoments) ? 0u : 1u;
  for (int i = 0; i < 7; i++) S.est[i] = est[i];
  if (converged) {
    S.termination = LOAMX_CONVERGED;
    S.active = 0;
  } else if (iteration + 1 >= C.max_iterations) {
    S.active = 0;
  } else {
    atomicAdd(B.n_active, 1u);
  }
}

__global__ __launch_bounds__(64) void lm_pair_loop_kernel(RegBatch B, RegConfig C) {
  __shared__ LightLds L;
  __shared__ double s_mom[kMomSize + 2];
  __shared__ double s_acc[kAccSize];
  __shared__ double s_edge[9][kEdgeCache];
  __shared__ double s_frec[7][kFlatCache];
  __shared__ uint32_t s_listed[kListCache], s_pref[kListCache];
  const int lane = threadIdx.x;
  const size_t pair = blockIdx.x;
  PairState& S_global = B.state[pair];
  if (!S_global.active) return;
  if (!S_global.lm.active) {
    if (lane == 0) outer_update_pair(B, C, pair, S_global);
    return;
  }
  __shared__ PairState s_S;
  static_assert(sizeof(PairState) % 8 == 0, "copied as 64-bit words");
  {
    const unsigned long long* __restrict__ src = reinterpret_cast<const unsigned long long*>(&S_global);
    unsigned long long* dst = reinterpret_cast<unsigned long long*>(&s_S);
    for (int w = lane; w < (int)(sizeof(PairState) / 8); w += 64) dst[w] = src[w];
  }
  wave_lds_fence();
  PairState& S = s_S;
  const uint32_t n_se_raw = B.n_src_edge[pair * B.in_pitch], n_sp_raw = B.n_src_planar[pair * B.in_pitch];
  const uint32_t n_se = n_se_raw < B.edge_stride ? n_se_raw : (uint32_t)B.edge_stride;
  const uint32_t n_sp = n_sp_raw < B.planar_stride ? n_sp_raw : (uint32_t)B.planar_stride;
  {
    const size_t efield = B.n_pairs * B.edge_stride;
    const double* __restrict__ E = B.assoc.edge + pair * B.edge_stride;
    const uint32_t nc = n_se < kEdgeCache ? n_se : kEdgeCache;
    for (uint32_t v = lane; v < nc; v += 64) {
#pragma unroll
      for (int f = 0; f < 9; f++) s_edge[f][v] = E[f * efield + v];
    }
    static_assert(kListCache == 64, "one lane per tile");
    s_listed[lane] = (uint32_t)lane < B.mom_blocks_per_pair * 4 ? B.flagged_count[pair * B.mom_blocks_per_pair * 4 + lane] : 0u;
  }
  uint32_t stream = 1u;
  if (S.use_moments) {
    uint32_t used = (n_sp + kSweepChunk - 1) / kSweepChunk;
    used = used < B.mom_blocks_per_pair ? used : B.mom_blocks_per_pair;
    const double* __restrict__ part = B.mom_partials + pair * B.mom_blocks_per_pair * 4 * (size_t)(kMomSize + 2);
    double* __restrict__ mom = B.moments + pair * (size_t)(kMomSize + 2);
    double v[kMomSize / 64];
#pragma unroll
    for (int c = 0; c < kMomSize / 64; c++) v[c] = 0.0;
    double s0max = 0.0, v2max = 0.0;
    constexpr uint32_t kTileBatch = 4;
    for (uint32_t t0 = 0; t0 < used * 4; t0 += kTileBatch) {
      double w[kTileBatch][kMomSize / 64], m0[kTileBatch], m1[kTileBatch];
#pragma unroll
      for (uint32_t b = 0; b < kTileBatch; b++) {
        const bool in = t0 + b < used * 4;
        const size_t off = (in ? t0 + b : t0) * (size_t)(kMomSize + 2);
#pragma unroll
        for (int c = 0; c < kMomSize / 64; c++) w[b][c] = in ? part[off + c * 64 + lane] : 0.0;
        m0[b] = in ? part[off + kMomSize] : 0.0, m1[b] = in ? part[off + kMomSize + 1] : 0.0;
      }
#pragma unroll
      for (uint32_t b = 0; b < kTileBatch; b++) {
#pragma unroll
        for (int c = 0; c < kMomSize / 64; c++) v[c] += w[b][c];
        s0max = fmax(s0max, m0[b]), v2max = fmax(v2max, m1[b]);
      }
    }
#pragma unroll
    for (int c = 0; c < kMomSize / 64; c++) mom[c * 64 + lane] = v[c], s_mom[c * 64 + lane] = v[c];
    if (lane == 0) mom[kMomSize] = s0max, mom[kMomSize + 1] = v2max, s_mom[kMomSize] = s0max, s_mom[kMomSize + 1] = v2max;
    const double ident[7] = {0, 0, 0, 1, 0, 0, 0};
    stream = (S.mom_ref_on ? plane_moments_valid_rel(s0max, v2max, S.lm.xeval, S.mom_ref) : plane_moments_valid_at(s0max, v2max, ident)) ? 0u : 1u;
  }
  if (lane == 0) S.stream_planes = stream;
  uint32_t n_flat = 0xFFFFFFFFu;
  if (S.use_moments && B.mom_blocks_per_pair * 4 <= kListCache) {
    const uint32_t tiles = B.mom_blocks_per_pair * 4;
    const uint32_t mine = ((uint32_t)lane < tiles && ((uint32_t)lane / 4) * kSweepChunk < n_sp) ? s_listed[lane] : 0u;
    uint32_t incl = mine;
#pragma unroll
    for (int off = 1; off < 64; off <<= 1) {
// ... 168 lines not shown
  out[pair].termination = S.termination;
  out[pair].iterations = S.iterations;
}

inline unsigned per_pair_grid(size_t n_pairs) { return (unsigned)((n_pairs + 63) / 64); }

template <bool PLANE, int KM>
__global__ __launch_bounds__(64) void fit_sets_kernel(const double* __restrict__ pts, size_t n_sets, int k, double* __restrict__ prim_out,
                                                      double* __restrict__ aux_out) {
  const size_t s = (size_t)blockIdx.x * 64 + threadIdx.x;
  if (s >= n_sets) return;
  Vec3 nb[KM];
#pragma unroll
  for (int j = 0; j < KM; j++) {
    const size_t at = (s * (size_t)k + (size_t)(j < k ? j : 0)) * 3;
    nb[j] = j < k ? v3(pts[at], pts[at + 1], pts[at + 2]) : v3(0, 0, 0);
  }
  if (PLANE) {
    Vec3 nrm;
    double d;
    aux_out[s] = fit_plane<KM>(nb, k, nrm, d);
    prim_out[4 * s] = nrm.x, prim_out[4 * s + 1] = nrm.y, prim_out[4 * s + 2] = nrm.z, prim_out[4 * s + 3] = d;
  } else {
    Vec3 a, b;
    fit_line<KM>(nb, k, a, b);
    aux_out[s] = kDblMax;
    prim_out[6 * s] = a.x, prim_out[6 * s + 1] = a.y, prim_out[6 * s + 2] = a.z;
    prim_out[6 * s + 3] = b.x, prim_out[6 * s + 4] = b.y, prim_out[6 * s + 5] = b.z;
  }
}

template <int KM>
__global__ __launch_bounds__(64) void knn_queries_kernel(GridSet gs, const double* __restrict__ q, size_t n_q, int k, double max_dist,
                                                         double pass_max, uint32_t* __restrict__ idx_out, uint32_t* __restrict__ count_out) {
  __shared__ uint32_t s_rows[kLeanRowWords * 64];
  const size_t i = (size_t)blockIdx.x * 64 + threadIdx.x;
  if (i >= n_q) return;
  const GridDesc g = gs.desc[0];
  uint32_t pos[KM];
  const int kk = k < KM ? k : KM;
  const Vec3 p = v3(q[3 * i], q[3 * i + 1], q[3 * i + 2]);
  int kept;
  if (g.n_points <= kBruteMax) {
    KnnResult<KM> r;
    knn_init(r);
    brute_scan_tile(r, kk, p, gs.sorted, 0u, g.n_points);
    kept = knn_finish(r, kk, max_dist);
    knn_shift_positions<KM>(r.pos, kk, pos);
  } else {
    kept = knn_search_positions<KM>(g, gs.cell_start, gs.sorted, p, kk, max_dist, pass_max, pos, s_rows + threadIdx.x, 64);
  }
  count_out[i] = (uint32_t)kept;
#pragma unroll
  for (int u = 0; u < KM; u++) {
    const int j = u - (KM - kk);
    if (j >= 0) idx_out[i * (size_t)k + j] = j < kept ? gs.sorted[pos[u]].orig : 0xFFFFFFFFu;
  }
  for (int j = KM; j < k; j++) idx_out[i * (size_t)k + j] = 0xFFFFFFFFu;
}

template <bool PLANE, int KM>
__global__ __launch_bounds__(256) void assoc_dump_kernel(RegBatch B, RegConfig C, AssocDumpSet D) {
  const size_t stride = PLANE ? B.planar_stride : B.edge_stride;
  const uint32_t n_raw = PLANE ? B.n_src_planar[0] : B.n_src_edge[0];
  const uint32_t n_src = n_raw < stride ? n_raw : (uint32_t)stride;
  const uint32_t queued = B.assoc.n_assoc[PLANE ? 3 : 2];
  const uint32_t t = blockIdx.x * 256 + threadIdx.x;
  if (t >= n_src + queued) return;
  const GridSet& gs = PLANE ? B.grid_plane : B.grid_edge;
  const GridSet& src_gs = PLANE ? B.src_grid_plane : B.src_grid_edge;
  const uint32_t* __restrict__ nn = PLANE ? B.assoc.nn_plane : B.assoc.nn_edge;
  const uint32_t* __restrict__ rnn = PLANE ? B.assoc.rnn_plane : B.assoc.rnn_edge;
  const uint32_t* __restrict__ rest = PLANE ? B.assoc.rest_plane : B.assoc.rest_edge;
  uint32_t i, at;
  const uint32_t* __restrict__ src;
  if (t < n_src) {
    i = t, at = t, src = nn;
    if (nn[t] == 0xFFFFFFFFu) return;
  } else {
    at = t - n_src, i = rest[at] & kQueueIndex, src = rnn;
  }
  const uint32_t orig = src_gs.sorted[i].orig;
  const int kq = PLANE ? C.k_plane : C.k_edge, kk = kq < KM ? kq : KM, shift = KM - kk;
  const uint32_t kept = src[at];
  D.nn_count[orig] = kept;
  for (int j = 0; j < kk; j++) {
    const uint32_t pos = src[(size_t)(1 + shift + j) * stride + at];
    D.nn_idx[(size_t)orig * (size_t)kq + j] = (uint32_t)j < kept && pos < gs.stride ? gs.sorted[pos].orig : 0xFFFFFFFFu;
  }
  const double* __restrict__ rec = PLANE ? B.assoc.plane : B.assoc.edge;
  const double f0 = rec[i];
  D.valid[orig] = f0 == f0 ? 1 : 0;
  const GridPoint sq = src_gs.sorted[i];
  const Vec3 p = pose_act(B.state[0].est, v3(sq.x, sq.y, sq.z));
  D.moved[3 * (size_t)orig] = p.x, D.moved[3 * (size_t)orig + 1] = rec[stride + i], D.moved[3 * (size_t)orig + 2] = rec[2 * stride + i];
  for (int f = 0; f < (PLANE ? 4 : 6); f++) D.prim[(size_t)orig * (PLANE ? 4 : 6) + f] = rec[(size_t)(3 + f) * stride + i];
}

}

void launch_fit_sets(bool plane, const double* d_pts, size_t n_sets, int k, double* d_prim, double* d_aux, hipStream_t s) {
  if (n_sets == 0) return;
  const dim3 grid((unsigned)((n_sets + 63) / 64));
  if (k <= 5) {
    if (plane) launch_kernel((fit_sets_kernel<true, 5>), grid, dim3(64), 0, s, d_pts, n_sets, k, d_prim, d_aux);
    else launch_kernel((fit_sets_kernel<false, 5>), grid, dim3(64), 0, s, d_pts, n_sets, k, d_prim, d_aux);
  } else if (k <= 8) {
    if (plane) launch_kernel((fit_sets_kernel<true, 8>), grid, dim3(64), 0, s, d_pts, n_sets, k, d_prim, d_aux);
    else launch_kernel((fit_sets_kernel<false, 8>), grid, dim3(64), 0, s, d_pts, n_sets, k, d_prim, d_aux);
  } else {
    if (plane) launch_kernel((fit_sets_kernel<true, kFitMaxK>), grid, dim3(64), 0, s, d_pts, n_sets, k, d_prim, d_aux);
    else launch_kernel((fit_sets_kernel<false, kFitMaxK>), grid, dim3(64), 0, s, d_pts, n_sets, k, d_prim, d_aux);
  }
}

void launch_knn_queries(const GridSet& gs, const double* d_q, size_t n_q, int k, double max_dist, uint32_t* d_idx, uint32_t* d_count,
                        hipStream_t s) {
  if (n_q == 0) return;
  const dim3 grid((unsigned)((n_q + 63) / 64));
  const double pass_max = knn_radius_pass_max(max_dist);
  if (k <= 5) launch_kernel((knn_queries_kernel<5>), grid, dim3(64), 0, s, gs, d_q, n_q, k, max_dist, pass_max, d_idx, d_count);
  else if (k <= 8) launch_kernel((knn_queries_kernel<8>), grid, dim3(64), 0, s, gs, d_q, n_q, k, max_dist, pass_max, d_idx, d_count);
  else launch_kernel((knn_queries_kernel<16>), grid, dim3(64), 0, s, gs, d_q, n_q, k, max_dist, pass_max, d_idx, d_count);
}

void launch_assoc_dump(const RegBatch& B, const RegConfig& C, const AssocDumpSet& edge, const AssocDumpSet& plane, hipStream_t s) {
  const dim3 ge((unsigned)((2 * B.edge_stride + 255) / 256)), gp((unsigned)((2 * B.planar_stride + 255) / 256));
  if (edge.nn_count) {
    if (C.k_edge <= 5) launch_kernel((assoc_dump_kernel<false, 5>), ge, dim3(256), 0, s, B, C, edge);
    else if (C.k_edge <= 8) launch_kernel((assoc_dump_kernel<false, 8>), ge, dim3(256), 0, s, B, C, edge);
    else launch_kernel((assoc_dump_kernel<false, 16>), ge, dim3(256), 0, s, B, C, edge);
  }
  if (plane.nn_count) {
    if (C.k_plane <= 5) launch_kernel((assoc_dump_kernel<true, 5>), gp, dim3(256), 0, s, B, C, plane);
    else if (C.k_plane <= 8) launch_kernel((assoc_dump_kernel<true, 8>), gp, dim3(256), 0, s, B, C, plane);
    else launch_kernel((assoc_dump_kernel<true, 16>), gp, dim3(256), 0, s, B, C, plane);
  }
}

static bool grid_big(size_t stride, const GridPoint* scratch, uint32_t flags) {
  return !grid_small(stride, flags) && scratch != nullptr && stride * sizeof(GridPoint) >= kBigScratchBytes && !(flags & kRegFlagNoBigGrid);
}
static void launch_grid_build_big(size_t n_pairs, const double* pts, const uint32_t* n_pts, size_t stride, uint32_t in_pitch,
                                  double max_dist, const GridSet& gs, GridPoint* scratch, hipStream_t s) {
  const dim3 chunks((unsigned)((stride + kBigChunk - 1) / kBigChunk), (unsigned)n_pairs);
  launch_kernel(gridbig_init_kernel, dim3((unsigned)n_pairs), dim3(64), 0, s, scratch, stride);
  launch_kernel(gridbig_bbox_kernel, chunks, dim3(kBigThreads), 0, s, pts, n_pts, stride, in_pitch, scratch);
  launch_kernel(gridbig_choose_kernel, dim3((unsigned)((n_pairs + 63) / 64)), dim3(64), 0, s, n_pts, stride, in_pitch, max_dist, gs,
                     scratch, n_pairs);
  (void)hipMemsetAsync(gs.cell_start, 0, (gs.cells_cap ? (size_t)gs.cells_cap + 1 : n_pairs * (size_t)(kGridCellsCap + 1)) * sizeof(uint32_t), s);
  launch_kernel(gridbig_pass_kernel<false>, chunks, dim3(kBigThreads), 0, s, pts, n_pts, stride, in_pitch, gs, scratch);
  const unsigned n_tiles = (unsigned)(((gs.cells_cap ? gs.cells_cap : kGridCellsCap) + 1 + kScanTile - 1) / kScanTile);
  launch_kernel(gridbig_tile_sum_kernel, dim3(n_tiles, (unsigned)n_pairs), dim3(kScanThreads), 0, s, stride, gs, scratch);
  launch_kernel(gridbig_tile_scan_kernel, dim3((unsigned)n_pairs), dim3(kScanThreads), 0, s, stride, gs, scratch);
  launch_kernel(gridbig_scan_kernel, dim3(n_tiles, (unsigned)n_pairs), dim3(kScanThreads), 0, s, n_pts, stride, in_pitch, gs, scratch);
  launch_kernel(gridbig_pass_kernel<true>, chunks, dim3(kBigThreads), 0, s, pts, n_pts, stride, in_pitch, gs, scratch);
  if (gs.rel)
    launch_kernel(gridbig_rel_kernel, dim3((unsigned)((stride + kGridPad + kBigThreads - 1) / kBigThreads), (unsigned)n_pairs), dim3(kBigThreads), 0,
                       s, n_pts, stride, in_pitch, gs);
}

size_t index_insert_ws_bytes(size_t cells, size_t n_add) {
  return 16 + (2 * (cells + 1) + n_add + (cells + 1 + kScanTile - 1) / kScanTile) * sizeof(uint32_t);
}
void launch_index_insert_count(const GridSet& gs, size_t cells, const double* d_add, uint32_t n_add, void* ws, hipStream_t s) {
  uint32_t* flag = static_cast<uint32_t*>(ws);
  uint32_t* shift = flag + 4;
// ... 138 lines not shown
    if (mode_ != 1u)                                                                                              \
      launch_kernel((associate_knn_brute_kernel<PL, KMV>), grid_, dim3(kAssocThreads), 0, (st), B, C, (nblk)); \
  } while (0)
#define LOAMX_ASSOC_A2(PL, KMV, nblk, st)                                                                         \
  launch_kernel((associate_fit_kernel<PL, KMV>), dim3((unsigned)(pair_groups * 8 * (nblk))), dim3(kAssocThreads), 0, \
                     (st), B, C, (nblk))
#define LOAMX_ASSOC_B(PL, KMV, nblk, st)                                                                          \
  do {                                                                                                            \
    const uint32_t rblk_ = rest_blocks(B.n_pairs, (nblk));                                                        \
    const uint32_t one_ = queue_one_stage(B, C, (PL)) ? 1u : 0u;                                                  \
    if (one_) {                                                                                                   \
      launch_kernel((associate_knn_rest_kernel<PL, KMV, true>), dim3((unsigned)(pair_groups * 8 * rblk_)),   \
                         dim3(kRestThreads), 0, (st), B, C, rblk_);                                               \
    } else {                                                                                                      \
      launch_kernel((associate_knn_rest_kernel<PL, KMV, false>), dim3((unsigned)(pair_groups * 8 * rblk_)),  \
                         dim3(kRestThreads), 0, (st), B, C, rblk_);                                               \
      if (!queue_leftovers_coop(C, (PL))) {                                                                       \
        launch_kernel((associate_knn_left_kernel<PL, KMV>), dim3((unsigned)(pair_groups * 8 * rblk_)),       \
                           dim3(kRestThreads), 0, (st), B, C, rblk_);                                             \
      } else {                                                                                                    \
        const uint32_t cblk_ = coop_blocks(B.n_pairs);                                                            \
        launch_kernel((associate_knn_coop_kernel<PL, KMV>), dim3((unsigned)(pair_groups * 8 * cblk_)),       \
                           dim3(kRestThreads), 0, (st), B, C, cblk_);                                             \
      }                                                                                                           \
    }                                                                                                             \
    launch_kernel((associate_fit_queued_kernel<PL, KMV>), dim3((unsigned)(pair_groups * 8 * rblk_)),         \
                       dim3(kRestThreads), 0, (st), B, C, rblk_);                                                 \
  } while (0)
#define LOAMX_ASSOC_K(STEP, PL, nblk, st)                \
  do {                                                   \
    if ((PL ? C.k_plane : C.k_edge) <= 5) STEP(PL, 5, nblk, st); \
    else if ((PL ? C.k_plane : C.k_edge) <= 8) STEP(PL, 8, nblk, st); \
    else STEP(PL, 16, nblk, st);                         \
  } while (0)
  const bool edges = (what & kAssocEdges) != 0u && be != 0u, planes = (what & kAssocPlanes) != 0u && bp != 0u;
  if (edges && planes && B.knn_mode_edge == 2u && B.knn_mode_plane == 1u && C.k_edge <= 5 && C.k_plane <= 5 &&
      !(C.flags & kRegFlagNoMixedAssoc)) {
    const uint32_t edge_blocks = (uint32_t)(pair_groups * 8 * be);
    const dim3 grid((unsigned)(edge_blocks + pair_groups * 8 * bp));
    LaunchScope* outer = g_launch_scope;
    if (knn_scope) g_launch_scope = knn_scope;
    launch_kernel((associate_knn_mixed_kernel<5, 5>), grid, dim3(kAssocThreads), 0, s, B, C, be, bp, edge_blocks);
    g_launch_scope = outer;
    hipStream_t sb = aux2 ? aux2 : aux;
    const bool fork2 = sb != nullptr && hipEventRecord(ev_mid, s) == hipSuccess && hipStreamWaitEvent(sb, ev_mid, 0) == hipSuccess;
    launch_kernel((associate_fit_mixed_kernel<5, 5>), grid, dim3(kAssocThreads), 0, s, B, C, be, bp, edge_blocks);
    LOAMX_ASSOC_B(true, 5, bp, (fork2 ? sb : s));
    if (fork2 && hipEventRecord(aux2 ? ev_join2 : ev_join, sb) == hipSuccess) (void)hipStreamWaitEvent(s, aux2 ? ev_join2 : ev_join, 0);
    return;
  }
  const bool use_aux = aux != nullptr && planes;
  const bool fork = use_aux && (edges || !aux2) && hipEventRecord(ev_fork, s) == hipSuccess &&
                    hipStreamWaitEvent(aux, ev_fork, 0) == hipSuccess;
  hipStream_t sa = fork ? aux : s;
  if (edges) {
    LOAMX_ASSOC_K(LOAMX_ASSOC_A1, false, be, sa);
    LOAMX_ASSOC_K(LOAMX_ASSOC_A2, false, be, sa);
    if (B.knn_mode_edge != 2u) LOAMX_ASSOC_K(LOAMX_ASSOC_B, false, be, sa);
  }
  if (planes) {
    LOAMX_ASSOC_K(LOAMX_ASSOC_A1, true, bp, s);
    hipStream_t sb = aux2 ? aux2 : aux;
    const bool fork2 = use_aux && (aux2 || fork) && hipEventRecord(ev_mid, s) == hipSuccess && hipStreamWaitEvent(sb, ev_mid, 0) == hipSuccess;
    LOAMX_ASSOC_K(LOAMX_ASSOC_A2, true, bp, s);
    if (B.knn_mode_plane != 2u) LOAMX_ASSOC_K(LOAMX_ASSOC_B, true, bp, (fork2 ? sb : s));
    if (fork2 && aux2 && hipEventRecord(ev_join2, aux2) == hipSuccess) (void)hipStreamWaitEvent(s, ev_join2, 0);
  }
  if (fork && hipEventRecord(ev_join, aux) == hipSuccess) (void)hipStreamWaitEvent(s, ev_join, 0);
#undef LOAMX_ASSOC_A1
#undef LOAMX_ASSOC_A2
#undef LOAMX_ASSOC_B
#undef LOAMX_ASSOC_K
}

#ifdef LOAMX_NN_SAME_STATS
__global__ void nn_same_kernel(RegBatch B, uint32_t* prev, unsigned long long* stats, uint32_t it) {
  const size_t pair = blockIdx.y;
  const uint32_t i = blockIdx.x * blockDim.x + threadIdx.x;
  const uint32_t n = B.n_src_planar[pair * B.in_pitch];
  if (i >= n || i >= B.planar_stride || !B.state[pair].active) return;
  const size_t field = B.n_pairs * B.planar_stride, slot = pair * B.planar_stride + i;
  bool same = it > 0, queued = B.assoc.nn_plane[slot] == 0xFFFFFFFFu;
  for (int f = 0; f < 6; f++) {
    const uint32_t v = B.assoc.nn_plane[f * field + slot];
    if (prev[f * field + slot] != v) same = false;
    prev[f * field + slot] = v;
  }
  atomicAdd(&stats[0], 1ull);
  if (same && !queued) atomicAdd(&stats[1], 1ull);
  if (queued) atomicAdd(&stats[2], 1ull);
}
void debug_nn_same(const RegBatch& B, uint32_t it, hipStream_t s) {
  static uint32_t* prev = nullptr;
  static unsigned long long* stats = nullptr;
  const size_t words = 6 * B.n_pairs * B.planar_stride;
  if (!prev) { (void)hipMalloc(&prev, words * 4); (void)hipMalloc(&stats, 24); }
  (void)hipMemsetAsync(stats, 0, 24, s);
  launch_kernel(nn_same_kernel, dim3((unsigned)((B.planar_stride + 255) / 256), (unsigned)B.n_pairs), dim3(256), 0, s, B, prev, stats, it);
  unsigned long long h[3];
  (void)hipMemcpyAsync(h, stats, 24, hipMemcpyDeviceToHost, s);
  (void)hipStreamSynchronize(s);
  printf("nn_same it=%u: %llu active plane queries, %llu keep their list (%.1f %%), %llu queued (%.1f %%)\n", it, h[0], h[1],
         100.0 * (double)h[1] / (double)(h[0] ? h[0] : 1), h[2], 100.0 * (double)h[2] / (double)(h[0] ? h[0] : 1));
}
#endif

void launch_sweep(const RegBatch& B, hipStream_t s) {
  if (B.n_pairs == 0 || B.blocks_per_pair == 0) return;
  launch_kernel(sweep_kernel, dim3((unsigned)(B.n_pairs * B.blocks_per_pair)), dim3(kSweepThreads), 0, s, B);
}

void launch_lm_pair_loop(const RegBatch& B, const RegConfig& C, hipStream_t s) {
  if (B.n_pairs == 0) return;
  launch_kernel(lm_pair_loop_kernel, dim3((unsigned)B.n_pairs), dim3(64), 0, s, B, C);
}

void launch_moments(const RegBatch& B, hipStream_t s) {
  if (B.n_pairs == 0 || B.mom_blocks_per_pair == 0) return;
  launch_kernel(moment_kernel, dim3((unsigned)(B.n_pairs * B.mom_blocks_per_pair * 4)), dim3(64), 0, s, B);
}

void launch_lm_step(const RegBatch& B, hipStream_t s) {
  if (B.n_pairs == 0) return;
  launch_kernel(lm_step_kernel, dim3(per_pair_grid(B.n_pairs)), dim3(64), 0, s, B);
}

void launch_lm_begin(const RegBatch& B, const RegConfig& C, hipStream_t s) {
  if (B.n_pairs == 0) return;
  launch_kernel(lm_begin_kernel, dim3(per_pair_grid(B.n_pairs)), dim3(64), 0, s, B, C);
}

void launch_outer_update(const RegBatch& B, const RegConfig& C, hipStream_t s) {
  if (B.n_pairs == 0) return;
  launch_kernel(outer_update_kernel, dim3(per_pair_grid(B.n_pairs)), dim3(64), 0, s, B, C);
}

void launch_write_results(const RegBatch& B, loamx_reg_result* d_results, hipStream_t s) {
  if (B.n_pairs == 0) return;
  launch_kernel(write_results_kernel, dim3(per_pair_grid(B.n_pairs)), dim3(64), 0, s, B, d_results);
}

}
```

Baseline: 102,100 pairs/s.

## Compact live pairs and bound KNN search window from previous kth distance

Keeps a double-buffered list of still-active pairs so per-pair kernels map their blocks onto live pairs only, instead of launching blocks that exit early for converged pairs. It also stores a rounded upper bound on each query's kth-neighbor distance alongside the kept count, and uses that bound plus the pose displacement to shrink the KNN search radius and x-cell range on later iterations. This aims to cut wasted blocks and grid cells scanned, in exchange for extra state, packed nn words, and more complex correctness reasoning about the bounds.

```diff
diff --git a/loam_amd/csrc/loamx_api.hip b/loam_amd/csrc/loamx_api.hip
--- a/loam_amd/csrc/loamx_api.hip
+++ b/loam_amd/csrc/loamx_api.hip
@@ -22,7 +22,7 @@
   WS_XYZ = 0, WS_CURV, WS_MASK, WS_EDGE_STAGE, WS_PLANAR_STAGE, WS_EDGE_CNT, WS_PLANAR_CNT,
   WS_EDGE_IDX, WS_PLANAR_IDX, WS_N_EDGE, WS_N_PLANAR, WS_EDGE_XYZ, WS_PLANAR_XYZ,
   WS_GRID_DESC_E, WS_GRID_DESC_P, WS_CELLS_E, WS_CELLS_P, WS_SORTED_E, WS_SORTED_P, WS_REL_E, WS_REL_P,
-  WS_SGRID_DESC_E, WS_SGRID_DESC_P, WS_SCELLS_E, WS_SCELLS_P, WS_SSORTED_E, WS_SSORTED_P, WS_SORT_SCRATCH, WS_SORT_SCRATCH_SRC, WS_ASSOC_E, WS_ASSOC_P, WS_NN_E, WS_NN_P, WS_RNN_E, WS_RNN_P, WS_NEAREST_E, WS_NEAREST_P, WS_REST_E, WS_REST_P, WS_EXACT_E, WS_EXACT_P, WS_NASSOC, WS_STATE, WS_PARTIALS, WS_MOM_PARTIALS, WS_MOMENTS, WS_FLAGGED_LIST, WS_FLAGGED_COUNT, WS_LINE_TOT, WS_EXTRACT_EVENTS, WS_BOX, WS_FINITE_FLAG,
+  WS_SGRID_DESC_E, WS_SGRID_DESC_P, WS_SCELLS_E, WS_SCELLS_P, WS_SSORTED_E, WS_SSORTED_P, WS_SORT_SCRATCH, WS_SORT_SCRATCH_SRC, WS_ASSOC_E, WS_ASSOC_P, WS_NN_E, WS_NN_P, WS_RNN_E, WS_RNN_P, WS_NEAREST_E, WS_NEAREST_P, WS_REST_E, WS_REST_P, WS_EXACT_E, WS_EXACT_P, WS_NASSOC, WS_STATE, WS_PARTIALS, WS_MOM_PARTIALS, WS_MOMENTS, WS_FLAGGED_LIST, WS_FLAGGED_COUNT, WS_LIVE, WS_LINE_TOT, WS_EXTRACT_EVENTS, WS_BOX, WS_FINITE_FLAG,
   WS_COUNTERS, WS_ITERINFO, WS_STREAM_IN0, WS_STREAM_IN1, WS_STREAM_RES, WS_DUMP_E, WS_DUMP_P, WS_FIT_IN, WS_FIT_OUT, WS_SRC_E, WS_SRC_P, WS_TGT_E, WS_TGT_P, WS_FCOUNTS, WS_RESULTS, WS_INIT,
   WS_COUNT
 };
@@ -119,7 +119,8 @@
     {"NO_MIXED_ASSOC", false, kRegFlagNoMixedAssoc}, {"FORCE_RCCL", false, kRegFlagForceRccl},
     {"NO_COOP_LEFT", false, kRegFlagNoCoopLeft}, {"NO_REF_MOMENTS", false, kRegFlagNoRefMoments},
     {"NO_EXTRACT_BOXES", false, kRegFlagNoExtractBoxes}, {"CHECK_FINITE", false, kRegFlagCheckFinite},
-    {"NO_SMALL_SETS", false, kRegFlagNoSmallSets}};
+    {"NO_SMALL_SETS", false, kRegFlagNoSmallSets}, {"NO_LIVE_LIST", false, kRegFlagNoLiveList},
+    {"NO_PREV_BOUND", false, kRegFlagNoPrevBound}};
 
 int fail(loamx_ctx* ctx, int code, const std::string& msg) {
   if (ctx) ctx->last_error = msg;
@@ -564,6 +565,7 @@
   ENSURE(ctx, WS_MOMENTS, np * (size_t)(kMomSize + 2) * sizeof(double));
   ENSURE(ctx, WS_FLAGGED_LIST, np * (size_t)B.mom_blocks_per_pair * kSweepChunk * sizeof(uint32_t));
   ENSURE(ctx, WS_FLAGGED_COUNT, np * (size_t)B.mom_blocks_per_pair * 4 * sizeof(uint32_t));
+  ENSURE(ctx, WS_LIVE, 2 * np * sizeof(uint32_t));
   {
     const bool fresh = ctx->ws[WS_COUNTERS].cap == 0;
     ENSURE(ctx, WS_COUNTERS, 128);
@@ -575,7 +577,7 @@
                                    WS_SGRID_DESC_E, WS_SGRID_DESC_P, WS_SCELLS_E, WS_SCELLS_P, WS_SSORTED_E, WS_SSORTED_P, WS_SORT_SCRATCH, WS_SORT_SCRATCH_SRC,
                                    WS_ASSOC_E, WS_ASSOC_P, WS_NN_E, WS_NN_P, WS_RNN_E, WS_RNN_P, WS_NEAREST_E, WS_NEAREST_P, WS_REST_E,
                                    WS_REST_P, WS_EXACT_E, WS_EXACT_P, WS_NASSOC, WS_STATE, WS_PARTIALS, WS_MOM_PARTIALS, WS_MOMENTS,
-                                   WS_FLAGGED_LIST, WS_FLAGGED_COUNT};
+                                   WS_FLAGGED_LIST, WS_FLAGGED_COUNT, WS_LIVE};
     for (int id : kScratch)
       if (ctx->ws[id].p) HIP_TRY(ctx, hipMemsetAsync(ctx->ws[id].p, 0xFF, ctx->ws[id].cap, ctx->stream));
   }
@@ -601,6 +603,9 @@
   B.flagged_list = wsp<uint32_t>(ctx, WS_FLAGGED_LIST);
   B.flagged_count = wsp<uint32_t>(ctx, WS_FLAGGED_COUNT);
   B.n_active = wsp<uint32_t>(ctx, WS_COUNTERS);
+  B.live = (C.flags & kRegFlagNoLiveList) ? nullptr : wsp<uint32_t>(ctx, WS_LIVE);
+  B.live_parity = 0u;
+  B.prev_bound = (C.flags & kRegFlagNoPrevBound) ? 0u : 1u;
   B.sweep_slots = reinterpret_cast<unsigned long long*>(wsp<unsigned char>(ctx, WS_COUNTERS) + 8);
   B.assoc_slots = B.sweep_slots + 2;
   B.grid_bytes = B.sweep_slots + 5;
@@ -680,13 +685,14 @@
     return LOAMX_OK;
   }
   for (uint32_t it = 0; it < C.max_iterations; it++) {
+    B.live_parity = it & 1u;
     {
       const int rc_body = enqueue_icf_iteration(ctx, B, C, it, hook, hook_user);
       if (rc_body != LOAMX_OK) return rc_body;
     }
     if (it + 1 < C.max_iterations && it > (B.n_pairs >= 256 ? 1u : 0u)) {
       untimed(ctx);
-      HIP_TRY(ctx, hipMemcpyAsync(ctx->h_pinned, B.n_active, sizeof(uint32_t), hipMemcpyDeviceToHost, s));
+      HIP_TRY(ctx, hipMemcpyAsync(ctx->h_pinned, B.n_active + (B.live_parity ^ 1u), sizeof(uint32_t), hipMemcpyDeviceToHost, s));
       launch_write_results(B, d_results, s);
       CHECK_LAUNCH(ctx, "write_results_kernel");
       HIP_TRY(ctx, hipStreamSynchronize(s));
diff --git a/loam_amd/csrc/loamx_internal.h b/loam_amd/csrc/loamx_internal.h
--- a/loam_amd/csrc/loamx_internal.h
+++ b/loam_amd/csrc/loamx_internal.h
@@ -114,6 +114,8 @@
 constexpr uint32_t kRegFlagNoSmallSets = 8192u;
 constexpr uint32_t kRegFlagCheckFinite = 4096u;
 constexpr uint32_t kRegFlagNoExtractBoxes = 2048u;
+constexpr uint32_t kRegFlagNoLiveList = 16384u;
+constexpr uint32_t kRegFlagNoPrevBound = 32768u;
 constexpr uint32_t kRegFlagNoMixedAssoc = 128u;
 
 struct GridSet {
@@ -152,6 +154,7 @@
   uint32_t use_moments;
   uint32_t mom_ref_on;
   double mom_ref[7];
+  float disp[2];
 };
 
 constexpr int kSweepThreads = 256;
@@ -188,6 +191,9 @@
   uint32_t* flagged_count;
   uint32_t blocks_per_pair;
   uint32_t* n_active;
+  uint32_t* live;
+  uint32_t live_parity;
+  uint32_t prev_bound;
   unsigned long long* sweep_slots;
   unsigned long long* assoc_slots;
   unsigned long long* grid_bytes;
diff --git a/loam_amd/csrc/reg_math.h b/loam_amd/csrc/reg_math.h
--- a/loam_amd/csrc/reg_math.h
+++ b/loam_amd/csrc/reg_math.h
@@ -938,7 +938,7 @@
 template <int KM, int W = 1>
 LOAMX_HD int knn_lean_finish(const GridDesc& g, const GridPoint* __restrict__ sp, Vec3 q, int k, double max_dist, double pass_max,
                              double a, int32_t cx, int32_t cy, int32_t cz, const KnnKeys32<KM>& c, uint64_t started,
-                             const uint32_t* row_scratch, int row_stride, int vis_off, uint32_t pos[KM]) {
+                             const uint32_t* row_scratch, int row_stride, int vis_off, uint32_t pos[KM], float* kth_up = nullptr) {
   constexpr uint32_t imask = 0xFFu;
   constexpr int NR = (2 * W + 1) * (2 * W + 1);
   {
@@ -1000,15 +1000,19 @@
     }
   }
   const uint32_t k6 = c.key[KM];
-  if (count == k && k6 != 0xFFFFFFFFu) {
-    const double t6 = (double)knn_bits_f32(k6 & ~imask);
+  if (count == k) {
 #if defined(__HIP_DEVICE_COMPILE__)
-    const double sd5 = (double)(__fsqrt_rn((float)d5) * 1.000001f) + 1e-18;
-#else
-    const double sd5 = (double)(sqrtf((float)d5) * 1.000001f) + 1e-18;
-#endif
-    const double err = 2.0 * (3.4641016151377544 * a * sd5 + 3.0 * a * a + 2.384185791015625e-7 * d5);
-    if (!(t6 > d5 + err)) undecided = true;
+    const float sd5f = __fsqrt_rn((float)d5) * 1.000001f;
+#else
+    const float sd5f = sqrtf((float)d5) * 1.000001f;
+#endif
+    if (kth_up) *kth_up = sd5f;
+    if (k6 != 0xFFFFFFFFu) {
+      const double t6 = (double)knn_bits_f32(k6 & ~imask);
+      const double sd5 = (double)sd5f + 1e-18;
+      const double err = 2.0 * (3.4641016151377544 * a * sd5 + 3.0 * a * a + 2.384185791015625e-7 * d5);
+      if (!(t6 > d5 + err)) undecided = true;
+    }
   }
   if (undecided) LOAMX_LEAN_REASON(2);
   return undecided ? -3 : kept;
@@ -1056,7 +1060,8 @@
 template <int KM, typename Requery = KnnSameQuery>
 LOAMX_HD int knn_lean_round1(const GridDesc& g, const uint32_t* __restrict__ cell_start, const GridPoint* __restrict__ sp,
                              const float* __restrict__ rel, uint32_t plane, Vec3 q, int k, double max_dist, double pass_max,
-                             uint32_t pos[KM], uint32_t* row_scratch, int row_stride, Requery requery = Requery()) {
+                             uint32_t pos[KM], uint32_t* row_scratch, int row_stride, Requery requery = Requery(),
+                             float w_prior = 3.0e38f, float* kth_up = nullptr) {
 #pragma unroll
   for (int j = 0; j < KM; j++) pos[j] = 0;
   if (g.n_points == 0 || k <= 0) return 0;
@@ -1075,11 +1080,18 @@
   const double sz2m = slab_dist(q.z, g.oz, g.h, cz - 1), sz2p = slab_dist(q.z, g.oz, g.h, cz + 1);
   const float fy2[3] = {(float)(sy2m * sy2m) * kDown, 0.0f, (float)(sy2p * sy2p) * kDown};
   const float fz2[3] = {(float)(sz2m * sz2m) * kDown, 0.0f, (float)(sz2p * sz2p) * kDown};
-  const float fr2 = r2 < 1e37 ? (float)r2 * kUp : 3.0e38f;
+  float fr2 = r2 < 1e37 ? (float)r2 * kUp : 3.0e38f;
   const float fa2 = (float)(3003.0 * a * a) * kUp;
   int nrow = 0;
   {
-    const int32_t xa = cx - 1 < 0 ? 0 : cx - 1, xb = cx + 1 > g.nx - 1 ? g.nx - 1 : cx + 1;
+    int32_t xa = cx - 1 < 0 ? 0 : cx - 1, xb = cx + 1 > g.nx - 1 ? g.nx - 1 : cx + 1;
+    if (w_prior < 1.5f * (float)g.h) {
+      const float w2 = w_prior * w_prior * kUp;
+      fr2 = w2 < fr2 ? w2 : fr2;
+      const double wd = (double)w_prior;
+      const int32_t xl = grid_cell_coord(q.x - wd, g.ox, g.inv_h), xh = grid_cell_coord(q.x + wd, g.ox, g.inv_h);
+      xa = xl > xa ? xl : xa, xb = xh < xb ? xh : xb;
+    }
     uint32_t rb[9], re[9];
 #pragma unroll
     for (int o = 0; o < 9; o++) {
@@ -1178,7 +1190,7 @@
   {
     const Vec3 q2 = requery(q);
     const int32_t cx2 = grid_cell_coord(q2.x, g.ox, g.inv_h), cy2 = grid_cell_coord(q2.y, g.oy, g.inv_h), cz2 = grid_cell_coord(q2.z, g.oz, g.inv_h);
-    return knn_lean_finish<KM>(g, sp, q2, k, max_dist, pass_max, a, cx2, cy2, cz2, c, started, row_scratch, row_stride, 0, pos);
+    return knn_lean_finish<KM>(g, sp, q2, k, max_dist, pass_max, a, cx2, cy2, cz2, c, started, row_scratch, row_stride, 0, pos, kth_up);
   }
 }
 
@@ -1302,10 +1314,11 @@
 LOAMX_HD int knn_search_f32_round1(const GridDesc& g, const uint32_t* __restrict__ cell_start,
                                    const GridPoint* __restrict__ sp, const float* __restrict__ rel, uint32_t plane, Vec3 q,
                                    int k, double max_dist, double pass_max, uint32_t pos[KM], uint32_t* row_scratch,
-                                   int row_stride, Requery requery = Requery()) {
+                                   int row_stride, Requery requery = Requery(), float w_prior = 3.0e38f, float* kth_up = nullptr) {
 #if !defined(LOAMX_NO_LEAN_KNN)
   if (!WIDE && g.n_points <= kLeanMaxPoints)
-    return knn_lean_round1<KM>(g, cell_start, sp, rel, plane, q, k, max_dist, pass_max, pos, row_scratch, row_stride, requery);
+    return knn_lean_round1<KM>(g, cell_start, sp, rel, plane, q, k, max_dist, pass_max, pos, row_scratch, row_stride, requery, w_prior,
+                               kth_up);
 #endif
 #pragma unroll
   for (int j = 0; j < KM; j++) pos[j] = 0;
@@ -2058,6 +2071,25 @@
   st.active = lm_propose(st) ? 1 : 0;
 }
 
+LOAMX_HD void knn_displacement_bound(const double old[7], const double next[7], float out[2]) {
+  double f2 = 0.0;
+  for (int j = 0; j < 3; j++) {
+    const Vec3 e = v3(j == 0 ? 1.0 : 0.0, j == 1 ? 1.0 : 0.0, j == 2 ? 1.0 : 0.0);
+    const Vec3 d = vsub(quat_rotate(next, e), quat_rotate(old, e));
+    f2 += vdot(d, d);
+  }
+  const double n2 = 1.0 + (next[0] * next[0] + next[1] * next[1] + next[2] * next[2] + next[3] * next[3]) +
+                    (old[0] * old[0] + old[1] * old[1] + old[2] * old[2] + old[3] * old[3]);
+  const Vec3 dt = v3(next[4] - old[4], next[5] - old[5], next[6] - old[6]);
+  const double tn = 1.0 + vnorm(v3(next[4], next[5], next[6])) + vnorm(v3(old[4], old[5], old[6]));
+  out[0] = (float)(sqrt(f2) * (1.0 + 1e-6) + 1e-11 * n2);
+  out[1] = (float)(vnorm(dt) * (1.0 + 1e-6) + 1e-11 * tn);
+}
+LOAMX_HD float knn_prev_bound(float kth_prev, const float disp[2], double sx, double sy, double sz) {
+  const float s1 = (float)(fabs(sx) + fabs(sy) + fabs(sz));
+  return (kth_prev + (disp[0] * s1 + disp[1])) * 1.00001f;
+}
+
 LOAMX_HD bool outer_update(double est[7], const double update[7], double rot_thresh, double pos_thresh) {
   double next[7];
   pose_compose(update, est, next);
diff --git a/loam_amd/csrc/register_kernels.hip b/loam_amd/csrc/register_kernels.hip
--- a/loam_amd/csrc/register_kernels.hip
+++ b/loam_amd/csrc/register_kernels.hip
@@ -613,7 +613,10 @@
   S.use_moments = 0;
   S.mom_ref_on = 0;
   S.lm.active = 0;
+  S.disp[0] = S.disp[1] = __int_as_float(0x7F800000);
   for (int c = 0; c < 6; c++) B.assoc.n_assoc[8 * pair + c] = 0;
+  if (B.live) B.live[pair] = (uint32_t)pair;
+  if (pair == 0) B.n_active[0] = (uint32_t)B.n_pairs;
   if (B.max_counts) {
     const uint32_t ne = B.n_src_edge[pair * B.in_pitch], np = B.n_src_planar[pair * B.in_pitch];
     atomicMax(&B.max_counts[0], ne < B.edge_stride ? ne : (uint32_t)B.edge_stride);
@@ -638,15 +641,23 @@
 #define LOAMX_ASSOC_WAVES5 (LOAMX_KNN_REQUERY ? 6 : 4)
 #endif
 
-__device__ __forceinline__ bool xcd_pair_map(uint32_t block, uint32_t blocks_per_pair, size_t n_pairs, size_t& pair,
+__device__ __forceinline__ bool xcd_pair_map(uint32_t block, uint32_t blocks_per_pair, const RegBatch& B, size_t& pair,
                                              uint32_t& chunk) {
+  const size_t n_pairs = B.n_pairs;
   if (n_pairs < 8) {
     pair = block / blocks_per_pair;
     chunk = block % blocks_per_pair;
   } else {
     const uint32_t xcd = block & 7u, slot = block >> 3;
-    pair = (size_t)xcd + 8u * (size_t)(slot / blocks_per_pair);
+    const size_t rank = (size_t)xcd + 8u * (size_t)(slot / blocks_per_pair);
     chunk = slot % blocks_per_pair;
+    pair = rank;
+    if (B.live != nullptr) {
+      const uint32_t count = B.n_active[B.live_parity];
+      const uint32_t entry = B.live[(size_t)B.live_parity * n_pairs + (rank < n_pairs ? rank : n_pairs - 1)];
+      if (rank >= count) return false;
+      pair = entry;
+    }
   }
   return pair < n_pairs;
 }
@@ -670,12 +681,18 @@
   }
 }
 
+__device__ __forceinline__ uint32_t nn_word(int kept, float kth_up) {
+  return kept < 0 ? 0xFFFFFFFFu : (((__float_as_uint(kth_up) + 0xFFu) & ~0xFFu) | (uint32_t)kept);
+}
+__device__ __forceinline__ int nn_word_count(uint32_t w) { return (int)(int8_t)(w & 0xFFu); }
+__device__ __forceinline__ float nn_word_kth(uint32_t w) { return __uint_as_float(w & ~0xFFu); }
+
 template <bool PLANE, int KM>
 __device__ __forceinline__ void knn_brute_body(const RegBatch& B, const RegConfig& C, uint32_t blocks_per_pair, uint32_t block,
                                                GridPoint* s_tile) {
   size_t pair;
   uint32_t chunk;
-  if (!xcd_pair_map(block, blocks_per_pair, B.n_pairs, pair, chunk)) return;
+  if (!xcd_pair_map(block, blocks_per_pair, B, pair, chunk)) return;
   const PairState& S = B.state[pair];
   if (!S.active) return;
   const GridSet& gs = PLANE ? B.grid_plane : B.grid_edge;
@@ -797,7 +814,7 @@
   if (!has) return;
   const size_t field = B.n_pairs * stride, slot = pair * stride + i;
   uint32_t* __restrict__ nn = PLANE ? B.assoc.nn_plane : B.assoc.nn_edge;
-  nn[slot] = (uint32_t)kept;
+  nn[slot] = nn_word(kept, __int_as_float(0x7F800000));
 #pragma unroll
   for (int j = 0; j < KM; j++) nn[(1 + j) * field + slot] = pos[j];
 }
@@ -814,7 +831,7 @@
                                                 uint32_t* s_rows) {
   size_t pair;
   uint32_t chunk;
-  if (!xcd_pair_map(block, blocks_per_pair, B.n_pairs, pair, chunk)) return;
+  if (!xcd_pair_map(block, blocks_per_pair, B, pair, chunk)) return;
   const uint32_t i = chunk * kAssocThreads + threadIdx.x;
   const PairState& S = B.state[pair];
   if (!S.active) return;
@@ -833,6 +850,10 @@
   const GridPoint* __restrict__ sp = gs.sorted + pair * gs.stride;
   uint32_t pos[KM];
   const float* __restrict__ rel = gs.rel + pair * 3 * gs.stride;
+  uint32_t* __restrict__ nn = PLANE ? B.assoc.nn_plane : B.assoc.nn_edge;
+  float w_prior = 3.0e38f, kth_now = __int_as_float(0x7F800000);
+  if (B.prev_bound != 0u && S.iterations > 0u && S.disp[1] < 0.25f * (float)g.h)
+    w_prior = knn_prev_bound(nn_word_kth(nn[pair * stride + i]), S.disp, sq.x, sq.y, sq.z);
 #if LOAMX_KNN_REQUERY
   const GridPoint* __restrict__ src_pts = src_gs.sorted + pair * src_gs.stride;
   auto requery = [&](const Vec3&) -> Vec3 {
@@ -843,15 +864,14 @@
   };
   const int kept = knn_search_f32_round1<KM, false, decltype(requery)>(g, cs, sp, rel, (uint32_t)gs.stride, p, PLANE ? C.k_plane : C.k_edge,
                                              PLANE ? C.r_plane : C.r_edge, PLANE ? C.pass_plane : C.pass_edge, pos,
-                                             s_rows + threadIdx.x, kAssocThreads, requery);
+                                             s_rows + threadIdx.x, kAssocThreads, requery, w_prior, &kth_now);
 #else
   const int kept = knn_search_f32_round1<KM>(g, cs, sp, rel, (uint32_t)gs.stride, p, PLANE ? C.k_plane : C.k_edge,
                                              PLANE ? C.r_plane : C.r_edge, PLANE ? C.pass_plane : C.pass_edge, pos,
-                                             s_rows + threadIdx.x, kAssocThreads);
+                                             s_rows + threadIdx.x, kAssocThreads, KnnSameQuery(), w_prior, &kth_now);
 #endif
   const size_t field = B.n_pairs * stride, slot = pair * stride + i;
-  uint32_t* __restrict__ nn = PLANE ? B.assoc.nn_plane : B.assoc.nn_edge;
-  nn[slot] = kept < 0 ? 0xFFFFFFFFu : (uint32_t)kept;
+  nn[slot] = nn_word(kept, kth_now);
   if (kept < 0) {
     const uint32_t at = atomicAdd(&B.assoc.n_assoc[8 * pair + (PLANE ? 3 : 2)], 1u);
     (PLANE ? B.assoc.rest_plane : B.assoc.rest_edge)[pair * stride + at] = i | (kept == -2 ? kQueueWide : kept == -3 ? kQueueTied : 0u);
@@ -893,7 +913,7 @@
   constexpr bool one_stage = ONE_STAGE;
   size_t pair;
   uint32_t chunk0;
-  if (!xcd_pair_map(blockIdx.x, blocks_per_pair, B.n_pairs, pair, chunk0)) return;
+  if (!xcd_pair_map(blockIdx.x, blocks_per_pair, B, pair, chunk0)) return;
   const PairState& S = B.state[pair];
   if (!S.active) return;
   const uint32_t queued = B.assoc.n_assoc[8 * pair + (PLANE ? 3 : 2)];
@@ -947,7 +967,7 @@
                                                                                               uint32_t blocks_per_pair) {
   size_t pair;
   uint32_t chunk0;
-  if (!xcd_pair_map(blockIdx.x, blocks_per_pair, B.n_pairs, pair, chunk0)) return;
+  if (!xcd_pair_map(blockIdx.x, blocks_per_pair, B, pair, chunk0)) return;
   const PairState& S = B.state[pair];
   if (!S.active) return;
   const uint32_t listed = B.assoc.n_assoc[8 * pair + (PLANE ? 5 : 4)];
@@ -1155,7 +1175,7 @@
 __global__ __launch_bounds__(kRestThreads, LOAMX_COOP_WAVES) void associate_knn_coop_kernel(RegBatch B, RegConfig C, uint32_t blocks_per_pair) {
   size_t pair;
   uint32_t chunk0;
-  if (!xcd_pair_map(blockIdx.x, blocks_per_pair, B.n_pairs, pair, chunk0)) return;
+  if (!xcd_pair_map(blockIdx.x, blocks_per_pair, B, pair, chunk0)) return;
   const PairState& S = B.state[pair];
   if (!S.active) return;
   const uint32_t listed = B.assoc.n_assoc[8 * pair + (PLANE ? 5 : 4)];
@@ -1227,7 +1247,7 @@
   const Vec3 p = pose_act(S.est, v3(sq.x, sq.y, sq.z));
   const GridPoint* __restrict__ sp = gs.sorted + pair * gs.stride;
   const size_t field = B.n_pairs * stride, slot = pair * stride + i;
-  const int kept = (int)nnsrc[nidx];
+  const int kept = nn_word_count(nnsrc[nidx]);
   const int kq = PLANE ? C.k_plane : C.k_edge;
   const int shift = KM - (kq < KM ? kq : KM);
   double prim[6] = {0, 0, 0, 0, 0, 0};
@@ -1275,7 +1295,7 @@
 __device__ __forceinline__ void fit_body(const RegBatch& B, const RegConfig& C, uint32_t blocks_per_pair, uint32_t block) {
   size_t pair;
   uint32_t chunk;
-  if (!xcd_pair_map(block, blocks_per_pair, B.n_pairs, pair, chunk)) return;
+  if (!xcd_pair_map(block, blocks_per_pair, B, pair, chunk)) return;
   const uint32_t i = chunk * kAssocThreads + threadIdx.x;
   const PairState& S = B.state[pair];
   if (!S.active) return;
@@ -1303,7 +1323,7 @@
 __global__ __launch_bounds__(kRestThreads, 3) void associate_fit_queued_kernel(RegBatch B, RegConfig C, uint32_t blocks_per_pair) {
   size_t pair;
   uint32_t chunk0;
-  if (!xcd_pair_map(blockIdx.x, blocks_per_pair, B.n_pairs, pair, chunk0)) return;
+  if (!xcd_pair_map(blockIdx.x, blocks_per_pair, B, pair, chunk0)) return;
   const PairState& S = B.state[pair];
   if (!S.active) return;
   const uint32_t queued = B.assoc.n_assoc[8 * pair + (PLANE ? 3 : 2)];
@@ -1327,7 +1347,7 @@
 __global__ __launch_bounds__(64) void lm_begin_kernel(RegBatch B, RegConfig C) {
   const size_t pair = (size_t)blockIdx.x * blockDim.x + threadIdx.x;
   if (pair >= B.n_pairs) return;
-  if (pair == 0) *B.n_active = 0u;
+  if (pair == 0) B.n_active[B.live_parity ^ 1u] = 0u;
   PairState& S = B.state[pair];
   if (!S.active) return;
   const uint32_t iteration = S.iterations;
@@ -1645,9 +1665,10 @@
     for (int i = 0; i < 7; i++) I.estimate_update[i] = upd[i];
   }
   S.iterations = iteration + 1;
-  double est[7];
-  for (int i = 0; i < 7; i++) est[i] = S.est[i];
+  double est[7], old[7];
+  for (int i = 0; i < 7; i++) est[i] = old[i] = S.est[i];
   const bool converged = outer_update(est, upd, C.rot_thresh, C.pos_thresh);
+  knn_displacement_bound(old, est, S.disp);
   S.use_moments = (C.flags & kRegFlagNoMoments) ? 0u : 1u;
   for (int i = 0; i < 7; i++) S.est[i] = est[i];
   if (converged) {
@@ -1656,7 +1677,8 @@
   } else if (iteration + 1 >= C.max_iterations) {
     S.active = 0;
   } else {
-    atomicAdd(B.n_active, 1u);
+    const uint32_t at = atomicAdd(&B.n_active[B.live_parity ^ 1u], 1u);
+    if (B.live) B.live[(size_t)(B.live_parity ^ 1u) * B.n_pairs + at] = (uint32_t)pair;
   }
 }
 
@@ -1991,7 +2013,7 @@
   }
   const uint32_t orig = src_gs.sorted[i].orig;
   const int kq = PLANE ? C.k_plane : C.k_edge, kk = kq < KM ? kq : KM, shift = KM - kk;
-  const uint32_t kept = src[at];
+  const uint32_t kept = (uint32_t)nn_word_count(src[at]);
   D.nn_count[orig] = kept;
   for (int j = 0; j < kk; j++) {
     const uint32_t pos = src[(size_t)(1 + shift + j) * stride + at];
@@ -2296,7 +2318,7 @@
   const size_t field = B.n_pairs * B.planar_stride, slot = pair * B.planar_stride + i;
   bool same = it > 0, queued = B.assoc.nn_plane[slot] == 0xFFFFFFFFu;
   for (int f = 0; f < 6; f++) {
-    const uint32_t v = B.assoc.nn_plane[f * field + slot];
+    const uint32_t v = f == 0 ? (uint32_t)nn_word_count(B.assoc.nn_plane[slot]) : B.assoc.nn_plane[f * field + slot];
     if (prev[f * field + slot] != v) same = false;
     prev[f * field + slot] = v;
   }
```

Result: no change. 102,400 pairs/s (median of 6 runs) (+0.3%).
